# aiforvision/OCTA-autosegmentation

Measured on AMD Instinct MI355X. Metric: synthetic OCTA samples/sec (graph + 304x304 image + 1216x1216 label triples), higher is better.
Workload: dtype f64

## Files before the change

include/octa_hip.h:

```cpp
#ifndef OCTA_HIP_H
#define OCTA_HIP_H

#include <stddef.h>
#include <stdint.h>

#ifdef __cplusplus
extern "C" {
#endif

typedef struct octa_ctx octa_ctx;


int octa_abi_version(void);

const char *octa_last_error(void);

int octa_ctx_create(int device, octa_ctx **out);
void octa_ctx_destroy(octa_ctx *ctx);

size_t octa_ctx_scratch_bytes(const octa_ctx *ctx);

int octa_rasterize_2d(octa_ctx *ctx, int B, const double *d_edges, const int64_t *h_edge_off,
                      const uint8_t *d_keep, int no_pixels_x, int no_pixels_y, int mip_axis,
                      double min_radius, double max_radius, uint8_t *d_out, void *stream);
// ... 129 lines not shown

int octa_menten_vessel_noise(octa_ctx *ctx, const void *d_img, int img_dtype, const unsigned char *d_bernoulli, const double *d_quantum,
                             const double *d_weights, int radius, double scaling, double r, int B, int H, int W, double *d_tmp, double *d_out,
                             void *stream);
int octa_menten_floater_mask(octa_ctx *ctx, const int *d_pts, const int *d_npts, const int *d_dilations, int B, int P, int N,
                             unsigned char *d_mask, int *d_dist, void *stream);
int octa_menten_floater(octa_ctx *ctx, const double *d_img, const int *d_pts, const int *d_npts, const int *d_dilations, const double *d_weights,
                        int radius, int B, int P, int N, unsigned char *d_mask, int *d_dist, double *d_tmp, double *d_out, void *stream);
int octa_menten_motion(octa_ctx *ctx, const void *d_in, void *d_out, int elem_size, const int *d_table, const void *d_white, int n_white,
                       int unit_elems, int B, int H, int W, void *stream);

int octa_noise_model(octa_ctx *ctx, const float *d_img, const float *d_background, const float *d_grids, int B, int H, int W, int gh, int gw,
                     uint64_t seed, uint32_t sample_offset, double lambda_delta, double lambda_speckle, double lambda_gamma,
                     const float *d_delta_in, const float *d_n_in, float *d_out, float *d_maps, float *d_fields, void *stream);
void octa_philox4x32_10(const uint32_t *counter4, const uint32_t *key2, uint32_t *out4);

int octa_noise_model_backward(octa_ctx *ctx, const float *d_dout, const float *d_img, const float *d_background, const float *d_grids, int B, int H,
                              int W, int gh, int gw, uint64_t seed, uint32_t sample_offset, double lambda_delta, double lambda_speckle,
                              double lambda_gamma, const float *d_delta_in, const float *d_n_in, float *d_dgrids, float *d_dmaps, float *d_out,
                              float *d_maps, float *d_logodds, float *d_bgrad, void *stream);

int octa_conv3x3_c1_fwd(octa_ctx *ctx, const void *d_x, const float *d_w, void *d_y, int N, int H, int W, int Cout, double *d_stat, int nslot,
                        void *stream);
int octa_conv3x3_c1_wgrad(octa_ctx *ctx, const void *d_x, const void *d_dy, float *d_dw, int N, int H, int W, int Cout, void *stream);

int octa_dice_bce_fwd(octa_ctx *ctx, const void *d_logits, int dtype, const float *d_y, int B, int64_t n, double *d_sums, void *stream);
int octa_dice_bce_finish(octa_ctx *ctx, const double *d_sums, int B, int64_t n, double smooth_nr, double smooth_dr, float *d_loss, void *stream);
int octa_dice_bce_bwd(octa_ctx *ctx, const void *d_logits, int dtype, const float *d_y, int B, int64_t n, const double *d_sums,
                      const float *d_grad_out, float smooth_nr, float smooth_dr, void *d_dlogits, void *stream);

int octa_thinconv_expand(octa_ctx *ctx, const void *d_s, const void *d_w, const void *d_bias, void *d_out, int N, int Hs, int Ws, int C, int K,
                         int pad, int flip, float slope, void *stream);
int octa_thinconv_squeeze(octa_ctx *ctx, const void *d_a, const void *d_w, const void *d_bias, void *d_out, int N, int Ha, int Wa, int C, int K,
                          int pad, int flip, void *stream);
long long octa_thinconv_wgrad_scratch_floats(int N, int Ha, int C, int K);
int octa_lrelu_bwd_bf16(octa_ctx *ctx, const void *d_y, const void *d_dy, void *d_out, int64_t n, float slope, void *stream);
int octa_thinconv_wgrad(octa_ctx *ctx, const void *d_a, const void *d_s, void *d_scratch, void *d_g, void *d_asum, int N, int Ha, int Wa, int Hs,
                        int Ws, int C, int K, int pad, int flip, void *stream);

int octa_reflect_pad_fwd(octa_ctx *ctx, const void *d_in, void *d_out, int dtype, int B, int H, int W, int C, int pad, void *stream);
int octa_reflect_pad_bwd(octa_ctx *ctx, const void *d_in, void *d_out, int dtype, int B, int H, int W, int C, int pad, void *stream);
int octa_blur_down_fwd(octa_ctx *ctx, const void *d_in, void *d_out, int dtype, int B, int H, int W, int C, void *stream);
int octa_blur_down_bwd(octa_ctx *ctx, const void *d_in, void *d_out, int dtype, int B, int H, int W, int C, void *stream);
int octa_blur_up_fwd(octa_ctx *ctx, const void *d_in, void *d_out, int dtype, int B, int H, int W, int C, void *stream);
int octa_blur_up_bwd(octa_ctx *ctx, const void *d_in, void *d_out, int dtype, int B, int H, int W, int C, void *stream);

int octa_remove_small_objects(octa_ctx *ctx, const uint8_t *d_in, int B, int H, int W, int min_size, int connectivity,
                              uint8_t on_value, uint8_t *d_out, void *stream);

int octa_skeletonize(octa_ctx *ctx, const uint8_t *d_in, int B, int H, int W, uint8_t *d_out, int *passes, void *stream);


size_t octa_fft2_c2c_f64_workspace_bytes(int b, int h, int w);

int octa_fft2_c2c_f64(const void *d_in, void *d_out, int b, int h, int w, int inverse, void *d_ws, void *stream);

size_t octa_oof_workspace_bytes(int b, int h, int w);

int octa_oof_2d(const float *d_in, double *d_out, int b, int h, int w, void *d_ws, void *stream);

int octa_oof_2d_response(const float *d_in, double *d_out, int b, int h, int w, void *d_ws, void *stream);


size_t octa_frangi_workspace_bytes(int b, int h, int w, int n_scales);

int octa_frangi_2d(const float *d_in, double *d_out, int b, int h, int w, int n_scales, const int *radii, const double *weights, float in_scale,
                   double beta, double gamma, int black_ridges, void *d_ws, void *stream);

int octa_frangi_hessian(const float *d_in, float *d_hrr, float *d_hrc, float *d_hcc, int b, int h, int w, int radius, const double *weights,
                        float in_scale, int black_ridges, void *d_ws, void *stream);

int octa_frangi_eigenvalues(const float *d_in, float *d_l1, float *d_l2, float *d_gamma, int b, int h, int w, int radius, const double *weights,
                            float in_scale, int black_ridges, void *d_ws, void *stream);

typedef struct octa_sim octa_sim;

typedef struct {
    double param_scale, d, r;
    double faz_radius_mean, faz_radius_std;
    double rotation_radius;
    double faz_center[2];
    double size[3];
    int n_trees;
    int walls[4];
    int n_modes;
    double modes[8][13];
    int forest_type;
    double nerve_center[2];
    double nerve_radius;
    const uint8_t *geometry;
    int geometry_shape[3];
    int n_source_walls;
    int source_walls[6];
} octa_sim_config;

#define OCTA_BIF_MAX_ATTS 256
typedef struct {
    int sample, n;
    double pos[3];
    double r, kappa, d;
    double atts[OCTA_BIF_MAX_ATTS * 3];
} octa_bif_request;

typedef void (*octa_bif_fn)(int n_req, const octa_bif_request *reqs, double *out6, void *user);

int octa_bif_native_init(const char *blas_path, int n_kappa, const double *kappas, const double *cs, const double *sn,
                         octa_bif_fn fallback, void *fallback_user);
void octa_bif_native(int n_req, const octa_bif_request *reqs, double *out6, void *user);
int octa_bif_native_counts(int64_t *h_out2);

int octa_sim_create(octa_ctx *ctx, const octa_sim_config *cfg, int B, octa_sim **out);
int octa_sim_create_ex(octa_ctx *ctx, const octa_sim_config *cfg, int B, int build, octa_sim **out);
void octa_sim_destroy(octa_sim *sim);

long long octa_sim_launch_count(void);
int octa_order_wait_launch(octa_ctx *ctx, long long ticket, int timeout_us, int settle_us, int *d_out3, void *stream);

int octa_sim_run(octa_sim *sim, const uint32_t *h_np_seeds, const uint64_t *h_py_seeds, octa_bif_fn bif, void *user,
                 void *stream);

int octa_sim_run_states(octa_sim *sim, const double *h_faz_radius, const double *h_stumps, const uint32_t *h_np_states,
                        const uint32_t *h_py_states, octa_bif_fn bif, void *user, void *stream);
int octa_sim_np_state(octa_sim *sim, int sample, uint32_t *h_state625);

int octa_sim_edge_offsets(octa_sim *sim, int64_t *h_edge_off, int64_t *h_n_art);

int octa_sim_export_edges(octa_sim *sim, double *h_edges);

int octa_sim_export_edges_device(octa_sim *sim, double *d_edges, void *stream);

int octa_sim_trace(octa_sim *sim, int32_t *h_trace);

int octa_sim_stats(octa_sim *sim, int64_t *h_stats);

int octa_sim_kd_paths(octa_sim *sim, int64_t *h_paths);

int octa_sim_assign_paths(octa_sim *sim, int64_t *h_paths);

int octa_sim_spans(octa_sim *sim, int64_t *h_spans);

int octa_sim_timing(octa_sim *sim, double *h_out8);

int octa_sim_service_stats(octa_sim *sim, double *h_out5);

int octa_sim_geometry(int num_cus, int *h_out4);

int octa_sim_is_large(const octa_sim *sim);

int octa_sim_fields(octa_sim *sim, int sample, double *h_oxy, int64_t cap_oxy, int64_t *n_oxy, double *h_co2,
                    int64_t cap_co2, int64_t *n_co2);

int octa_sim_kat_kd_order(octa_ctx *ctx, const double *h_pts, int64_t n, const uint8_t *h_need, int32_t *h_indices);

#ifdef __cplusplus
}
#endif
#endif
```

octa_autosegmentation_amd/_native.py:

```python
import contextlib
import ctypes
import os
import random as _random
import threading

import numpy as np

HERE = os.path.dirname(os.path.abspath(__file__))
LIB_PATH = os.environ.get("OCTA_HIP_LIB") or os.path.join(HERE, "liboctahip.so")

_lib = None
_ctxs = {}
_lock = threading.Lock()

c_void_p, c_int, c_double, c_size_t = ctypes.c_void_p, ctypes.c_int, ctypes.c_double, ctypes.c_size_t


def _struct(name, ints, ptrs):
    fields = [("struct_size", ctypes.c_uint32)] + [(k, c_int) for k in ints.split()] + [("slope", ctypes.c_float)] + [(k, c_void_p) for k in ptrs.split()]
    return type(name, (ctypes.Structure,), {"_fields_": fields})


Conv3x3Args = _struct("Conv3x3Args", "N H W Cin Cout stride in_dilation tap_mask out_scale out_off_y out_off_x C1 CY1 nslot",
                      "d_x d_x2 d_w d_y d_y2 d_scale1 d_shift1 d_scale2 d_shift2 d_stat_partials d_stat_slots d_residual")
Conv3x3WgradArgs = _struct("Conv3x3WgradArgs", "N H W Cin Cout stride tap_mask C1 out_mode", "d_x d_x2 d_dy d_dw d_scale1 d_shift1 d_scale2 d_shift2")
WGRAD_TAP_MAJOR, WGRAD_PARAM_ADD, WGRAD_PARAM_SET = 0, 1, 2

SIGNATURES = {
    "octa_abi_version": (c_int, []),
    "octa_last_error": (ctypes.c_char_p, []),
    "octa_ctx_create": (c_int, [c_int, ctypes.POINTER(c_void_p)]),
    "octa_ctx_destroy": (None, [c_void_p]),
    "octa_ctx_scratch_bytes": (c_size_t, [c_void_p]),
    "octa_rasterize_2d": (c_int, [c_void_p, c_int, c_void_p, c_void_p, c_void_p, c_int, c_int, c_int, c_double,
                                  c_double, c_void_p, c_void_p]),
    "octa_rasterize_2d_plan": (c_int, [c_void_p, c_int, c_void_p, c_void_p, c_void_p, c_int, c_int, c_int, c_double, c_double, c_void_p]),
    "octa_rasterize_2d_draw": (c_int, [c_void_p, c_void_p, c_void_p]),
    "octa_raster_prof": (c_int, [c_void_p, c_void_p]),
    "octa_fs_dither": (c_int, [c_void_p, c_int, c_void_p, c_int, c_int, c_void_p, c_void_p]),
    "octa_voxel_padded_dims": (c_int, [c_void_p, c_void_p]),
    "octa_voxelize_3d": (c_int, [c_void_p, c_int, c_void_p, c_void_p, c_void_p, c_void_p, c_double, c_double, c_int, c_void_p, c_void_p]),
    "octa_edges_read_back": (c_int, [c_void_p, c_void_p, c_void_p, ctypes.c_int64, c_void_p, c_void_p]),
    "octa_max_u8": (c_int, [c_void_p, c_void_p, c_void_p, c_void_p, c_size_t, c_void_p]),
    "octa_bif_native_init": (c_int, [ctypes.c_char_p, c_int, c_void_p, c_void_p, c_void_p, c_void_p, c_void_p]),
    "octa_bif_native": (None, [c_int, c_void_p, c_void_p, c_void_p]),
    "octa_bif_native_counts": (c_int, [c_void_p]),
    "octa_instnorm_lrelu_fwd": (c_int, [c_void_p] * 7 + [c_int, c_int, ctypes.c_int64, c_int, ctypes.c_float, ctypes.c_float, c_void_p]),
    "octa_instnorm_lrelu_bwd": (c_int, [c_void_p] * 10 + [c_int, c_int, ctypes.c_int64, c_int, ctypes.c_float, c_void_p]),
    "octa_csv_bytes_bound": (ctypes.c_int64, [ctypes.c_int64]),
    "octa_csv_format_edges": (ctypes.c_int64, [c_void_p, ctypes.c_int64, c_void_p, ctypes.c_int64]),
    "octa_csv_write_file": (c_int, [ctypes.c_char_p, c_void_p, ctypes.c_int64]),
    "octa_csv_count_rows": (ctypes.c_int64, [c_void_p, ctypes.c_int64]),
    "octa_csv_parse_edges": (ctypes.c_int64, [c_void_p, ctypes.c_int64, c_void_p, ctypes.c_int64]),
    "octa_py_random_advance": (c_int, [c_void_p, ctypes.c_int64]),
    "octa_png_write_gray8": (c_int, [ctypes.c_char_p, c_void_p, c_int, c_int, c_int]),
    "octa_png_write_bits": (c_int, [ctypes.c_char_p, c_void_p, c_int, c_int, c_int]),
    "octa_write_sample_files": (c_int, [ctypes.c_int64, c_void_p, c_void_p, c_void_p, c_void_p, c_void_p, c_int, c_int, c_void_p, c_int, c_int, c_int,
                                        ctypes.c_char_p, ctypes.c_int64, c_int, c_int]),
    "octa_pack_bits": (c_int, [c_void_p, c_void_p, c_void_p, ctypes.c_int64, c_int, c_void_p]),
    "octa_background_noise": (c_int, [c_void_p, c_void_p, c_void_p, c_void_p, ctypes.c_int64, c_void_p, c_void_p, c_void_p]),
    "octa_speckle_brightness": (c_int, [c_void_p, c_void_p, c_void_p, c_void_p, c_int, c_int, c_int, c_void_p, c_void_p, c_void_p]),
    "octa_menten_vessel_noise": (c_int, [c_void_p, c_void_p, c_int, c_void_p, c_void_p, c_void_p, c_int, c_double, c_double, c_int, c_int, c_int, c_void_p, c_void_p, c_void_p]),
    "octa_menten_floater_mask": (c_int, [c_void_p, c_void_p, c_void_p, c_void_p, c_int, c_int, c_int, c_void_p, c_void_p, c_void_p]),
    "octa_menten_floater": (c_int, [c_void_p, c_void_p, c_void_p, c_void_p, c_void_p, c_void_p, c_int, c_int, c_int, c_int, c_void_p, c_void_p, c_void_p, c_void_p, c_void_p]),
    "octa_menten_motion": (c_int, [c_void_p, c_void_p, c_void_p, c_int, c_void_p, c_void_p, c_int, c_int, c_int, c_int, c_int, c_void_p]),
    "octa_noise_model": (c_int, [c_void_p, c_void_p, c_void_p, c_void_p, c_int, c_int, c_int, c_int, c_int, ctypes.c_uint64, ctypes.c_uint32, c_double, c_double, c_double,
                                 c_void_p, c_void_p, c_void_p, c_void_p, c_void_p, c_void_p]),
    "octa_noise_model_backward": (c_int, [c_void_p, c_void_p, c_void_p, c_void_p, c_void_p, c_int, c_int, c_int, c_int, c_int, ctypes.c_uint64, ctypes.c_uint32,
                                          c_double, c_double, c_double, c_void_p, c_void_p, c_void_p, c_void_p, c_void_p, c_void_p, c_void_p, c_void_p, c_void_p]),
    "octa_philox4x32_10": (None, [c_void_p, c_void_p, c_void_p]),
    "octa_sim_create": (c_int, [c_void_p, c_void_p, c_int, ctypes.POINTER(c_void_p)]),
    "octa_sim_create_ex": (c_int, [c_void_p, c_void_p, c_int, c_int, ctypes.POINTER(c_void_p)]),
    "octa_sim_destroy": (None, [c_void_p]),
    "octa_sim_run": (c_int, [c_void_p, c_void_p, c_void_p, c_void_p, c_void_p, c_void_p]),
    "octa_sim_run_states": (c_int, [c_void_p, c_void_p, c_void_p, c_void_p, c_void_p, c_void_p, c_void_p, c_void_p]),
    "octa_sim_np_state": (c_int, [c_void_p, c_int, c_void_p]),
    "octa_thinconv_expand": (c_int, [c_void_p, c_void_p, c_void_p, c_void_p, c_void_p, c_int, c_int, c_int, c_int, c_int, c_int, c_int, ctypes.c_float, c_void_p]),
    "octa_thinconv_squeeze": (c_int, [c_void_p, c_void_p, c_void_p, c_void_p, c_void_p, c_int, c_int, c_int, c_int, c_int, c_int, c_int, c_void_p]),
    "octa_lrelu_bwd_bf16": (c_int, [c_void_p, c_void_p, c_void_p, c_void_p, ctypes.c_int64, ctypes.c_float, c_void_p]),
    "octa_thinconv_wgrad_scratch_floats": (ctypes.c_longlong, [c_int, c_int, c_int, c_int]),
    "octa_thinconv_wgrad": (c_int, [c_void_p, c_void_p, c_void_p, c_void_p, c_void_p, c_void_p, c_int, c_int, c_int, c_int, c_int, c_int, c_int, c_int, c_int, c_void_p]),
    "octa_sim_spans": (c_int, [c_void_p, c_void_p]),
    "octa_sim_edge_offsets": (c_int, [c_void_p, c_void_p, c_void_p]),
    "octa_sim_export_edges": (c_int, [c_void_p, c_void_p]),
    "octa_sim_export_edges_device": (c_int, [c_void_p, c_void_p, c_void_p]),
    "octa_sim_trace": (c_int, [c_void_p, c_void_p]),
    "octa_sim_stats": (c_int, [c_void_p, c_void_p]),
    "octa_sim_kd_paths": (c_int, [c_void_p, c_void_p]),
    "octa_sim_assign_paths": (c_int, [c_void_p, c_void_p]),
    "octa_sim_timing": (c_int, [c_void_p, c_void_p]),
    "octa_sim_service_stats": (c_int, [c_void_p, c_void_p]),
    "octa_sim_geometry": (c_int, [c_int, c_void_p]),
    "octa_sim_is_large": (c_int, [c_void_p]),
    "octa_conv2d_f32_nchw": (c_int, [c_void_p, c_void_p, c_void_p, c_void_p, c_void_p] + [c_int] * 14 + [c_void_p]),
    "octa_convtranspose2x2_f32_nchw": (c_int, [c_void_p, c_void_p, c_void_p, c_void_p, c_int, c_int, c_int, c_int, c_int, c_void_p]),
    "octa_conv2d_f32_dgrad_nchw": (c_int, [c_void_p, c_void_p, c_void_p, c_void_p] + [c_int] * 11 + [c_void_p]),
    "octa_conv2d_f32_wgrad_workspace": (c_int, [c_int] * 10 + [ctypes.POINTER(c_size_t)]),
    "octa_conv2d_f32_wgrad_nchw": (c_int, [c_void_p, c_void_p, c_void_p, c_void_p, c_void_p, c_void_p, c_size_t] + [c_int] * 10 + [c_void_p]),
    "octa_sim_fields": (c_int, [c_void_p, c_int, c_void_p, ctypes.c_int64, c_void_p, c_void_p, ctypes.c_int64, c_void_p]),
    "octa_instnorm_lrelu_nhwc_bwd": (c_int, [c_void_p, c_void_p, c_void_p, c_void_p, c_void_p, c_void_p, c_void_p, c_void_p, c_void_p, c_void_p, c_int, c_int, ctypes.c_int64, ctypes.c_float, c_void_p]),
    "octa_pack_conv_weights": (c_int, [c_void_p, c_void_p, c_int, c_void_p, c_void_p]),
    "octa_head1_nhwc_bwd": (c_int, [c_void_p, c_void_p, c_void_p, c_void_p, ctypes.c_int64, c_int, c_void_p, c_void_p, c_void_p, c_void_p]),
    "octa_instnorm_nhwc_stats": (c_int, [c_void_p, c_void_p, c_void_p, c_void_p, c_void_p, c_void_p, c_void_p, c_void_p, c_int, c_int, ctypes.c_int64, ctypes.c_float, c_void_p]),
    "octa_scale_shift_lrelu_nhwc": (c_int, [c_void_p, c_void_p, c_void_p, c_void_p, c_void_p, c_int, c_int, ctypes.c_int64, ctypes.c_float, c_void_p]),
    "octa_resize_bilinear": (c_int, [c_void_p, c_void_p, c_int, c_int, c_int, c_int, c_void_p, c_int, c_int, c_void_p, c_void_p, c_void_p]),
    "octa_resize_bilinear_bwd": (c_int, [c_void_p, c_void_p, c_int, c_int, c_int, c_int, c_int, c_void_p, c_void_p]),
    "octa_flip_rot90_rotate": (c_int, [c_void_p, c_void_p, c_void_p, c_int, c_int, c_void_p, c_void_p, c_void_p, ctypes.c_float, c_int, c_void_p]),
    "octa_remove_small_objects": (c_int, [c_void_p, c_void_p, c_int, c_int, c_int, c_int, c_int, ctypes.c_uint8, c_void_p, c_void_p]),
    "octa_skeletonize": (c_int, [c_void_p, c_void_p, c_int, c_int, c_int, c_void_p, ctypes.POINTER(c_int), c_void_p]),
    "octa_reflect_pad_fwd": (c_int, [c_void_p, c_void_p, c_void_p, c_int, c_int, c_int, c_int, c_int, c_int, c_void_p]),
    "octa_reflect_pad_bwd": (c_int, [c_void_p, c_void_p, c_void_p, c_int, c_int, c_int, c_int, c_int, c_int, c_void_p]),
    "octa_blur_down_fwd": (c_int, [c_void_p, c_void_p, c_void_p, c_int, c_int, c_int, c_int, c_int, c_void_p]),
    "octa_blur_down_bwd": (c_int, [c_void_p, c_void_p, c_void_p, c_int, c_int, c_int, c_int, c_int, c_void_p]),
    "octa_blur_up_fwd": (c_int, [c_void_p, c_void_p, c_void_p, c_int, c_int, c_int, c_int, c_int, c_void_p]),
    "octa_blur_up_bwd": (c_int, [c_void_p, c_void_p, c_void_p, c_int, c_int, c_int, c_int, c_int, c_void_p]),
    "octa_conv4x4_nhwc_fwd": (c_int, [c_void_p, c_void_p, c_void_p, c_void_p, c_int, c_int, c_int, c_int, c_int, c_int, c_void_p]),
    "octa_conv4x4_nhwc_wgrad": (c_int, [c_void_p, c_void_p, c_void_p, c_void_p, c_int, c_int, c_int, c_int, c_int, c_void_p]),
    "octa_dice_bce_fwd": (c_int, [c_void_p, c_void_p, c_int, c_void_p, c_int, ctypes.c_int64, c_void_p, c_void_p]),
    "octa_dice_bce_finish": (c_int, [c_void_p, c_void_p, c_int, ctypes.c_int64, c_double, c_double, c_void_p, c_void_p]),
    "octa_dice_bce_bwd": (c_int, [c_void_p, c_void_p, c_int, c_void_p, c_int, ctypes.c_int64, c_void_p, c_void_p, ctypes.c_float, ctypes.c_float, c_void_p, c_void_p]),
    "octa_sim_launch_count": (ctypes.c_longlong, []),
    "octa_order_wait_launch": (c_int, [c_void_p, ctypes.c_longlong, c_int, c_int, c_void_p, c_void_p]),
    "octa_conv3x3_c1_wgrad": (c_int, [c_void_p, c_void_p, c_void_p, c_void_p, c_int, c_int, c_int, c_int, c_void_p]),
    "octa_conv_stat_tiles": (c_int, [c_int, c_int]),
    "octa_instnorm_lrelu_head1_nhwc_bwd": (c_int, [c_void_p, c_void_p, c_void_p, c_void_p, c_void_p, c_void_p, c_void_p, c_void_p, c_void_p, c_void_p, c_void_p, c_void_p, c_void_p, c_int, c_int, ctypes.c_int64, ctypes.c_float, c_void_p]),
    "octa_conv3x3_s2t_nhwc": (c_int, [c_void_p, c_void_p, c_void_p, c_void_p, c_int, c_int, c_int, c_int, c_int, c_int, c_void_p, c_void_p]),
    "octa_conv3x3_nhwc_fwd": (c_int, [c_void_p, ctypes.POINTER(Conv3x3Args), c_void_p]),
    "octa_conv3x3_nhwc_wgrad": (c_int, [c_void_p, ctypes.POINTER(Conv3x3WgradArgs), c_void_p]),
    "octa_conv3x3_nhwc_fwd_pad": (c_int, [c_void_p, c_void_p, c_void_p, c_void_p, c_int, c_int, c_int, c_int, c_int, c_int, c_int, c_void_p, c_int, c_void_p]),
    "octa_conv3x3_nhwc_wgrad_pad": (c_int, [c_void_p, c_void_p, c_void_p, c_void_p, c_int, c_int, c_int, c_int, c_int, c_int, c_int, c_int, c_void_p]),
    "octa_instnorm_lrelu_nhwc_fwd": (c_int, [c_void_p] * 7 + [c_int, c_int, ctypes.c_int64, ctypes.c_float, ctypes.c_float, c_void_p, c_int, c_void_p, c_int, c_void_p]),
    "octa_instnorm_lrelu_head1_nhwc_fwd": (c_int, [c_void_p] * 9 + [c_int, c_int, ctypes.c_int64, ctypes.c_float, ctypes.c_float, c_void_p, c_int, c_void_p]),
    "octa_head1_nhwc_fwd": (c_int, [c_void_p, c_void_p, c_void_p, c_void_p, ctypes.c_int64, c_int, c_void_p, c_void_p]),
    "octa_conv3x3_c1_fwd": (c_int, [c_void_p, c_void_p, c_void_p, c_void_p, c_int, c_int, c_int, c_int, c_void_p, c_int, c_void_p]),
    "octa_fft2_c2c_f64_workspace_bytes": (c_size_t, [c_int, c_int, c_int]),
    "octa_fft2_c2c_f64": (c_int, [c_void_p, c_void_p, c_int, c_int, c_int, c_int, c_void_p, c_void_p]),
    "octa_oof_workspace_bytes": (c_size_t, [c_int, c_int, c_int]),
    "octa_oof_2d": (c_int, [c_void_p, c_void_p, c_int, c_int, c_int, c_void_p, c_void_p]),
    "octa_oof_2d_response": (c_int, [c_void_p, c_void_p, c_int, c_int, c_int, c_void_p, c_void_p]),
    "octa_frangi_workspace_bytes": (c_size_t, [c_int, c_int, c_int, c_int]),
    "octa_frangi_2d": (c_int, [c_void_p, c_void_p, c_int, c_int, c_int, c_int, c_void_p, c_void_p, ctypes.c_float, c_double, c_double, c_int, c_void_p, c_void_p]),
    "octa_frangi_hessian": (c_int, [c_void_p, c_void_p, c_void_p, c_void_p, c_int, c_int, c_int, c_int, c_void_p, ctypes.c_float, c_int, c_void_p, c_void_p]),
    "octa_frangi_eigenvalues": (c_int, [c_void_p, c_void_p, c_void_p, c_void_p, c_int, c_int, c_int, c_int, c_void_p, ctypes.c_float, c_int, c_void_p, c_void_p]),
    "octa_sim_kat_kd_order": (c_int, [c_void_p, c_void_p, ctypes.c_int64, c_void_p, c_void_p]),
}


class OctaHipError(RuntimeError):
    pass


def lib():
    global _lib
    if _lib is None:
        with _lock:
            if _lib is None:
                if not os.path.exists(LIB_PATH):
                    raise OctaHipError(
                        f"{LIB_PATH} is missing: build it with `python -m octa_autosegmentation_amd.build` "
                        "(hipcc --offload-arch=gfx950). There is no CPU fallback.")
                import torch
                l = ctypes.CDLL(LIB_PATH)
                for name, (res, args) in SIGNATURES.items():
                    fn = getattr(l, name)
                    fn.restype = res
                    fn.argtypes = args
                _lib = l
    return _lib


_SYNC_DEBUG = bool(os.environ.get("OCTA_SYNC_DEBUG"))


def check(rc, what):
    if _SYNC_DEBUG and rc == 0:
        import sys
        import torch
        torch.cuda.current_stream().synchronize()
        print(f"[octa-sync] {threading.current_thread().name} {what} ok", file=sys.stderr, flush=True)
    if rc != 0:
        msg = lib().octa_last_error().decode("utf-8", "replace")
        raise OctaHipError(f"{what} failed (rc={rc}): {msg}")


_tls = threading.local()


def _device_index(device_index):
    import torch
    if not torch.cuda.is_available():
        raise OctaHipError("no ROCm GPU visible to torch; the HIP path cannot run (no CPU fallback)")
    return int(torch.cuda.current_device() if device_index is None else device_index)


def _create_ctx(device_index):
    out = c_void_p()
    call("octa_ctx_create", device_index, ctypes.byref(out))
    return out


def new_ctx(device_index=None):
    return _create_ctx(_device_index(device_index))


def free_ctx(h):
    if h is not None:
        lib().octa_ctx_destroy(h)


@contextlib.contextmanager
def use_ctx(h):
    prev = getattr(_tls, "ctx", None)
    _tls.ctx = h
    try:
        yield h
    finally:
        _tls.ctx = prev


def ctx(device_index=None):
    import torch
    if getattr(_tls, "ctx", None) is not None:
        return _tls.ctx
    device_index = _device_index(device_index)
    key = (device_index, threading.get_ident(), torch.cuda.current_stream(device_index).cuda_stream)
    with _lock:
        h = _ctxs.get(key)
    if h is None:
        h = _create_ctx(device_index)
        with _lock:
            _ctxs[key] = h
    return h


def current_stream_ptr():
    import torch
    return c_void_p(torch.cuda.current_stream().cuda_stream)


def addr(t):
    return t.data_ptr() if t is not None else None


def _ctx_of(device):
    return ctx(device.index)



def launch(name, device, *args, what=None, ctx=None, stream=None):
    argv = [_ctx_of(device) if ctx is None else ctx]
    for a in args:
        argv.append(a.data_ptr() if hasattr(a, "data_ptr") else a)
    argv.append(current_stream_ptr() if stream is None else stream)
    check(getattr(lib(), name)(*argv), what or name)


def call(name, *args, what=None):
    check(getattr(lib(), name)(*[a.data_ptr() if hasattr(a, "data_ptr") else a for a in args]), what or name)


def advance_python_random(n):
    if n <= 0:
        return
    if n < 64:
        for _ in range(n):
            _random.random()
        return
    ver, state, gauss = _random.getstate()
    arr = np.array(state, dtype=np.uint32)
    call("octa_py_random_advance", arr.ctypes.data, int(n))
    _random.setstate((ver, tuple(arr.tolist()), gauss))
```

octa_autosegmentation_amd/csrc/sim.hip:

```cpp

#include <chrono>
#include <vector>

#include "common.h"
#include "sim_host.h"
#include <thread>
#include <atomic>
#include <cstdlib>
#include <cstring>

using namespace OCTA_SIMK;

#if OCTA_SIM_LARGE
#define OCTA_SIM_T octa_simL_impl
#define OCTA_SIM_FN(name) octa_simL_##name
#else
#define OCTA_SIM_T octa_simS_impl
#define OCTA_SIM_FN(name) octa_simS_##name
#endif
#define octa_sim_create OCTA_SIM_FN(create)
#define octa_sim_destroy OCTA_SIM_FN(destroy)
#define octa_sim_run OCTA_SIM_FN(run)
#define octa_sim_run_states OCTA_SIM_FN(run_states)
#define octa_sim_np_state OCTA_SIM_FN(np_state)
#define octa_sim_edge_offsets OCTA_SIM_FN(edge_offsets)
#define octa_sim_export_edges OCTA_SIM_FN(export_edges)
#define octa_sim_export_edges_device OCTA_SIM_FN(export_edges_device)
#define octa_sim_trace OCTA_SIM_FN(trace)
#define octa_sim_stats OCTA_SIM_FN(stats)
#define octa_sim_kd_paths OCTA_SIM_FN(kd_paths)
#define octa_sim_assign_paths OCTA_SIM_FN(assign_paths)
#define octa_sim_fields OCTA_SIM_FN(fields)
#define octa_sim_service_stats OCTA_SIM_FN(service_stats)
#define octa_sim_geometry OCTA_SIM_FN(geometry)
#define octa_sim_spans OCTA_SIM_FN(spans)
#define octa_sim_timing OCTA_SIM_FN(timing)
#define octa_sim_kat_kd_order OCTA_SIM_FN(kat_kd_order)
struct OCTA_SIM_T;
extern "C" void octa_sim_destroy(OCTA_SIM_T *S);
extern "C" long long octa_sim_next_ticket(void);
extern "C" int *octa_sim_launch_flag(int device);

namespace {

constexpr int SIM_THREADS = SIM_THREADS_PER_WG;
constexpr int SIM_WG_PER_CU = 2;
#if OCTA_SIM_LARGE
constexpr size_t SIM_LDS = 2048;
#else
constexpr size_t SIM_LDS = SIM_LDS_BYTES;
static_assert((size_t)KD_MAILBOX_OFF + KD_MAILBOX_BYTES <= (size_t)SIM_USER_BYTES && SIM_WG_PER_CU * SIM_LDS <= 160 * 1024, "LDS budget");
#endif
static_assert((624 + 1248) * 4 <= SEQ_SIDE_LDS, "the Mersenne-Twister state and queue of the candidate stream fit the side-job LDS");
static_assert(SIM_THREADS == 64 * KD_WAVES, "kd mailboxes are sized for KD_WAVES waves");
constexpr int REQ_CAP = 8192;

static_assert(sizeof(BifRequest) == sizeof(octa_bif_request), "request layout must match the public header");
static_assert(MAXKEPT == OCTA_BIF_MAX_ATTS, "request capacity must match the public header");

struct BatchPtrs {
    double *npos[2], *nrad[2], *nkap[2];
    int *npar[2], *nch0[2], *nch1[2];
    unsigned char *nnch[2], *nact[2];
    double *oxy, *co2, *cand, *py_u;
    unsigned *py_state;
    int *nn, *act_list;
    int *nn_prev[2];
    double *nn_d2[2];
    unsigned *sorted;
    int *gnode, *gstart, *gcount;
    Rec *rec;
    int *glist, *child_group;
    FlushRec *fl_rec;
    idx_t *kd_idx, *kd_rank;
    unsigned char *removed, *ven_near;
    unsigned long long *hashes;
    unsigned *pairs;
    unsigned long long *set_hash;
    int *set_key, *tmp_int;
    double *grid_pts;
    unsigned *cand_idx;
    double *tmp_dbl;
    SampleScalars *sc;
    IterParams *iters;
    BifRequest *reqs;
    int *req_count;
    double *bif_results;
    unsigned *mt_state;
    unsigned short *valid;
    size_t valid_stride;
    unsigned *valid_count;
    int *n_per_iter;
    int *next_sample;
    unsigned char *wg_scratch;
#ifdef OCTA_SIM_DEBUG_SAT
    int *dbg;
#endif
    int *trace;
    int n_samples;
    SimConst C;
};

__device__ __forceinline__ SimArrays sample_arrays(const BatchPtrs &B, int s) {
    SimArrays A;
    for (int f = 0; f < 2; f++) {
        A.npos[f] = B.npos[f] + (size_t)s * NCAP * 3;
        A.nrad[f] = B.nrad[f] + (size_t)s * NCAP;
        A.nkap[f] = B.nkap[f] + (size_t)s * NCAP;
        A.npar[f] = B.npar[f] + (size_t)s * NCAP;
        A.nch0[f] = B.nch0[f] + (size_t)s * NCAP;
        A.nch1[f] = B.nch1[f] + (size_t)s * NCAP;
        A.nnch[f] = B.nnch[f] + (size_t)s * NCAP;
        A.nact[f] = B.nact[f] + (size_t)s * NCAP;
        A.nn_prev[f] = B.nn_prev[f] + (size_t)s * OCAP;
        A.nn_d2[f] = B.nn_d2[f] + (size_t)s * OCAP;
    }
    A.oxy = B.oxy + (size_t)s * OCAP * 3;
    A.co2 = B.co2 + (size_t)s * CCAP * 3;
    A.cand = B.cand + (size_t)s * NCANDCAP * 3;
    A.py_u = B.py_u + (size_t)s * PYCAP;
    A.nn = B.nn + (size_t)s * OCAP;
    A.act_list = B.act_list + (size_t)s * NCAP;
    A.sorted = B.sorted + (size_t)s * SORTCAP;
    A.gnode = B.gnode + (size_t)s * GCAP;
    A.gstart = B.gstart + (size_t)s * GCAP;
    A.gcount = B.gcount + (size_t)s * GCAP;
    A.rec = B.rec + (size_t)s * GCAP;
    A.glist = B.glist + (size_t)s * GCAP;
    A.child_group = B.child_group + (size_t)s * NCAP;
    A.fl_rec = B.fl_rec + (size_t)s * 2 * MURRAY_FLUSH_LDS;
    A.kd_idx = B.kd_idx + (size_t)s * OCAP;
    A.kd_rank = B.kd_rank + (size_t)s * OCAP;
    A.removed = B.removed + (size_t)s * OCAP;
    A.ven_near = B.ven_near + (size_t)s * OCAP;
    A.hashes = B.hashes + (size_t)s * OCAP;
    A.pairs = B.pairs + (size_t)s * PCAP;
    A.set_hash = B.set_hash + (size_t)s * SETCAP;
    A.set_key = B.set_key + (size_t)s * SETCAP;
    A.tmp_int = B.tmp_int + (size_t)s * (OCAP + 2 * NCANDCAP);
    A.grid_pts = B.grid_pts + (size_t)s * GRID_N * 3;
    A.tmp_dbl = B.tmp_dbl + (size_t)s * OCAP * 3;
    A.sc = B.sc + s;
#ifdef OCTA_SIM_DEBUG_SAT
    A.dbg = B.dbg ? B.dbg + (size_t)s * B.C.n_iter * 16 : nullptr;
    A.dbg_it = 0;
#endif
    return A;
}

struct WaveMt {
    unsigned *st;
    unsigned *ob;
    int cur, avail;
    int lane;
    __device__ void regen_block() {
        for (int c = 0; c < 623; c += 64) {
            int k = c + lane;
            unsigned nv = 0;
            if (k < 623) {
                unsigned y = (st[k] & 0x80000000u) | (st[k + 1] & 0x7fffffffu);
                unsigned m = (k < 227) ? st[k + 397] : st[k - 227];
                nv = m ^ (y >> 1) ^ ((y & 1u) ? 0x9908b0dfu : 0u);
            }
            __builtin_amdgcn_wave_barrier();
            if (k < 623) st[k] = nv;
            __builtin_amdgcn_wave_barrier();
        }
        if (lane == 0) {
            unsigned y = (st[623] & 0x80000000u) | (st[0] & 0x7fffffffu);
            st[623] = st[396] ^ (y >> 1) ^ ((y & 1u) ? 0x9908b0dfu : 0u);
        }
        __builtin_amdgcn_wave_barrier();
    }
    __device__ static unsigned temper(unsigned y) {
        y ^= (y >> 11);
        y ^= (y << 7) & 0x9d2c5680u;
        y ^= (y << 15) & 0xefc60000u;
        y ^= (y >> 18);
        return y;
    }
    __device__ void ensure(int k) {
        if (avail - cur >= k) return;
        const int rem = avail - cur;
        for (int c = 0; c < rem; c += 64) {
            int i = c + lane;
            unsigned v = (i < rem) ? ob[cur + i] : 0u;
            __builtin_amdgcn_wave_barrier();
            if (i < rem) ob[i] = v;
            __builtin_amdgcn_wave_barrier();
        }
// ... 942 lines not shown
            OCTA_HIP_CHECK(hipEventSynchronize(S->ev[1]));
            OCTA_HIP_CHECK(hipEventElapsedTime(&ms, S->ev[0], S->ev[1]));
            S->ms_a += ms; S->n_a++;
            break;
        }
        if (serve(0)) return -1;
        OCTA_HIP_CHECK(hipEventElapsedTime(&ms, S->ev[0], S->ev[1]));
        S->ms_a += ms; S->n_a++;
        OCTA_HIP_CHECK(hipEventRecord(S->ev[0], stream));
        hipLaunchKernelGGL(sim_iter_b_kernel, dim3((unsigned)B), dim3(SIM_THREADS), SIM_LDS, stream, P, it);
        OCTA_HIP_CHECK(hipGetLastError());
        OCTA_HIP_CHECK(hipEventRecord(S->ev[1], stream));
        if (serve(1)) return -1;
        OCTA_HIP_CHECK(hipEventElapsedTime(&ms, S->ev[0], S->ev[1]));
        S->ms_b += ms; S->n_b++;
    }
    S->ms_total = std::chrono::duration<double, std::milli>(std::chrono::steady_clock::now() - wall0).count();
    if (S->lockstep) {
        S->h_sc.resize(B);
        OCTA_HIP_CHECK(hipMemcpyAsync(S->h_sc.data(), P.sc, sizeof(SampleScalars) * B, hipMemcpyDeviceToHost, stream));
        OCTA_HIP_CHECK(hipStreamSynchronize(stream));
    }
    S->ran = true;
#ifdef OCTA_SIM_DEBUG_SAT
    if (const char *path = getenv("OCTA_SIM_DEBUG_DUMP")) {
        std::vector<int> h((size_t)B * S->iters.size() * 16);
        OCTA_HIP_CHECK(hipMemcpy(h.data(), P.dbg, h.size() * sizeof(int), hipMemcpyDeviceToHost));
        if (FILE *fp = fopen(path, "wb")) { fwrite(h.data(), sizeof(int), h.size(), fp); fclose(fp); }
    }
#endif
    for (int s = 0; s < B; s++)
        if (S->h_sc[s].err) {
            if ((S->h_sc[s].err & ERR_HOST_TIMEOUT) && !S->lockstep)
                octa::set_error("octa_sim_run: sample %d failed with capacity/error bits 0x%x: with parking disabled (OCTA_SIM_PARK_MS=0) a workgroup waited "
                                "more than %.0f ms for the host's mailbox answer (request ticket %d, answered %d, %ld tickets served this run, longest pass of the "
                                "service loop %.1f ms, longest bifurcation callback %.1f ms; the workgroup began waiting for ticket %ld at %.1f ms into its "
                                "launch, polled %ld times, at its deadline read answer %ld and its own request word back as %ld)", s, S->h_sc[s].err,
                                S->mail_timeout_ms, S->mail.req_ticket[s], S->mail.resp_ticket[s], S->diag_tickets, S->diag_max_gap_ms, S->diag_max_bif_ms,
                                S->h_sc[s].prof[13], S->h_sc[s].prof[12] * 1e-5, S->h_sc[s].prof[14], S->h_sc[s].prof[11], S->h_sc[s].prof[15]);
            else
                octa::set_error("octa_sim_run: sample %d failed with capacity/error bits 0x%x", s, S->h_sc[s].err);
            return -3;
        }
    return 0;
}
}

extern "C" int octa_sim_edge_offsets(OCTA_SIM_T *S, int64_t *h_edge_off, int64_t *h_n_art) {
    if (!S || !S->ran || !h_edge_off) { octa::set_error("octa_sim_edge_offsets: run the simulation first"); return -2; }
    h_edge_off[0] = 0;
    for (int s = 0; s < S->B; s++) {
        const SampleScalars &sc = S->h_sc[s];
        int64_t na = sc.n_nodes[0] - S->cfg.n_trees, nv = sc.n_nodes[1] - S->cfg.n_trees;
        h_edge_off[s + 1] = h_edge_off[s] + na + nv;
        if (h_n_art) h_n_art[s] = na;
    }
    return 0;
}

extern "C" int octa_sim_export_edges(OCTA_SIM_T *S, double *h_edges) {
    if (!S || !S->ran || !h_edges) { octa::set_error("octa_sim_export_edges: run the simulation first"); return -2; }
    OCTA_HIP_CHECK(hipSetDevice(S->ctx->device));
    const BatchPtrs &P = S->P;
    const int B = S->B;
    int nmax[2] = {0, 0};
    for (int s = 0; s < B; s++) for (int f = 0; f < 2; f++) nmax[f] = S->h_sc[s].n_nodes[f] > nmax[f] ? S->h_sc[s].n_nodes[f] : nmax[f];
    size_t need = 0;
    for (int f = 0; f < 2; f++) need += (size_t)B * nmax[f] * (24 + 8 + 4 + 4 + 4 + 1) + 64 * 6;
    if (S->export_cap < need) {
        if (S->export_stage) { hipError_t e = hipHostFree(S->export_stage); (void)e; S->export_stage = nullptr; S->export_cap = 0; }
        OCTA_HIP_CHECK(hipHostMalloc(&S->export_stage, need + need / 4));
        S->export_cap = need + need / 4;
    }
    hipStream_t stream = S->export_stream;
    if (!stream) { OCTA_HIP_CHECK(hipStreamCreateWithFlags(&S->export_stream, hipStreamNonBlocking)); stream = S->export_stream; }
    char *base = static_cast<char *>(S->export_stage);
    double *pos[2], *rad[2];
    int *par[2], *c0[2], *c1[2];
    unsigned char *nch[2];
    size_t off = 0;
    auto take = [&](size_t bytes) { char *p = base + off; off += (bytes + 63) & ~(size_t)63; return p; };
    for (int f = 0; f < 2; f++) {
        const size_t n = (size_t)nmax[f];
        pos[f] = reinterpret_cast<double *>(take((size_t)B * n * 24)); rad[f] = reinterpret_cast<double *>(take((size_t)B * n * 8));
        par[f] = reinterpret_cast<int *>(take((size_t)B * n * 4)); c0[f] = reinterpret_cast<int *>(take((size_t)B * n * 4));
        c1[f] = reinterpret_cast<int *>(take((size_t)B * n * 4)); nch[f] = reinterpret_cast<unsigned char *>(take((size_t)B * n));
        if (n == 0) continue;
        auto get = [&](void *dst, const void *src, size_t elem, size_t cap_elems) -> hipError_t {
            return hipMemcpy2DAsync(dst, n * elem, src, cap_elems * elem, n * elem, (size_t)B, hipMemcpyDeviceToHost, stream);
        };
        OCTA_HIP_CHECK(get(pos[f], P.npos[f], 24, NCAP)); OCTA_HIP_CHECK(get(rad[f], P.nrad[f], 8, NCAP));
        OCTA_HIP_CHECK(get(par[f], P.npar[f], 4, NCAP)); OCTA_HIP_CHECK(get(c0[f], P.nch0[f], 4, NCAP));
        OCTA_HIP_CHECK(get(c1[f], P.nch1[f], 4, NCAP)); OCTA_HIP_CHECK(get(nch[f], P.nnch[f], 1, NCAP));
    }
    OCTA_HIP_CHECK(hipStreamSynchronize(stream));
    long total = 0;
    for (int s = 0; s < B; s++) {
        const SampleScalars &sc = S->h_sc[s];
        const double *cp[2], *cr[2];
        const int *cpar[2], *cc0[2], *cc1[2];
        const unsigned char *cn[2];
        for (int f = 0; f < 2; f++) {
            const size_t n = (size_t)nmax[f];
            cp[f] = pos[f] + (size_t)s * n * 3; cr[f] = rad[f] + (size_t)s * n; cpar[f] = par[f] + (size_t)s * n;
            cc0[f] = c0[f] + (size_t)s * n; cc1[f] = c1[f] + (size_t)s * n; cn[f] = nch[f] + (size_t)s * n;
        }
        long n_art = 0;
        long ne = export_edges(cp, cr, cpar, cc0, cc1, cn, sc.n_nodes, S->cfg.n_trees, h_edges + 7 * total, 1L << 40, &n_art);
        if (ne < 0) { octa::set_error("octa_sim_export_edges: export failed"); return -1; }
        total += ne;
    }
    return 0;
}

extern "C" int octa_sim_export_edges_device(OCTA_SIM_T *S, double *d_edges, void *stream_) {
    if (!S || !S->ran || !d_edges) { octa::set_error("octa_sim_export_edges_device: run the simulation first"); return -2; }
    OCTA_HIP_CHECK(hipSetDevice(S->ctx->device));
    hipStream_t stream = (hipStream_t)stream_;
    const int B = S->B;
    std::vector<long> off(B + 1, 0);
    for (int s = 0; s < B; s++) off[s + 1] = off[s] + (S->h_sc[s].n_nodes[0] - S->cfg.n_trees) + (S->h_sc[s].n_nodes[1] - S->cfg.n_trees);
    if (!S->d_edge_off) OCTA_HIP_CHECK(hipMalloc(&S->d_edge_off, sizeof(long) * (B + 1)));
    OCTA_HIP_CHECK(hipMemcpyAsync(S->d_edge_off, off.data(), sizeof(long) * (B + 1), hipMemcpyHostToDevice, stream));
    OCTA_HIP_CHECK(hipStreamSynchronize(stream));
    const size_t lds = OCTA_SIM_LARGE ? 2048 : 2048 + (size_t)NCAP * 2 * sizeof(idx_t);
    hipLaunchKernelGGL(sim_export_kernel, dim3((unsigned)B, 2), dim3(256), lds, stream, S->P, S->d_edge_off, S->cfg.n_trees, d_edges);
    OCTA_HIP_CHECK(hipGetLastError());
    return 0;
}

extern "C" int octa_sim_trace(OCTA_SIM_T *S, int32_t *h_trace) {
    if (!S || !S->ran || !h_trace) { octa::set_error("octa_sim_trace: run the simulation first"); return -2; }
    OCTA_HIP_CHECK(hipSetDevice(S->ctx->device));
    OCTA_HIP_CHECK(hipMemcpy(h_trace, S->P.trace, sizeof(int32_t) * (size_t)S->B * S->iters.size() * 4, hipMemcpyDeviceToHost));
    return 0;
}

extern "C" int octa_sim_stats(OCTA_SIM_T *S, int64_t *h_stats) {
    if (!S || !S->ran || !h_stats) { octa::set_error("octa_sim_stats: run the simulation first"); return -2; }
    for (int s = 0; s < S->B; s++) {
        const SampleScalars &sc = S->h_sc[s];
        int64_t *o = h_stats + 32 * s;
        o[0] = sc.err; o[1] = sc.py_pos; o[2] = sc.murray_steps; o[3] = sc.n_bif; o[4] = sc.respec;
        o[5] = sc.n_nodes[0]; o[6] = sc.n_nodes[1];
        memcpy(&o[7], &sc.faz_radius, 8);
        for (int k = 0; k < 16; k++) o[8 + k] = sc.prof[k];
        for (int k = 0; k < 8; k++) o[24 + k] = sc.kdprof[k];
    }
    return 0;
}

extern "C" int octa_sim_kd_paths(OCTA_SIM_T *S, int64_t *h_paths) {
    if (!S || !S->ran || !h_paths) { octa::set_error("octa_sim_kd_paths: run the simulation first"); return -2; }
    for (int s = 0; s < S->B; s++) { h_paths[2 * s] = S->h_sc[s].kd_path[0]; h_paths[2 * s + 1] = S->h_sc[s].kd_path[1]; }
    return 0;
}

extern "C" int octa_sim_assign_paths(OCTA_SIM_T *S, int64_t *h_paths) {
    if (!S || !S->ran || !h_paths) { octa::set_error("octa_sim_assign_paths: run the simulation first"); return -2; }
    for (int s = 0; s < S->B; s++) { h_paths[2 * s] = S->h_sc[s].assign_path[0]; h_paths[2 * s + 1] = S->h_sc[s].assign_path[1]; }
    return 0;
}

extern "C" int octa_sim_fields(OCTA_SIM_T *S, int sample, double *h_oxy, int64_t cap_oxy, int64_t *n_oxy, double *h_co2,
                               int64_t cap_co2, int64_t *n_co2) {
    if (!S || !S->ran || sample < 0 || sample >= S->B) { octa::set_error("octa_sim_fields: bad arguments"); return -2; }
    OCTA_HIP_CHECK(hipSetDevice(S->ctx->device));
    const SampleScalars &sc = S->h_sc[sample];
    if (n_oxy) *n_oxy = sc.n_oxy;
    if (n_co2) *n_co2 = sc.n_co2;
    if (h_oxy) {
        int64_t n = sc.n_oxy < cap_oxy ? sc.n_oxy : cap_oxy;
        OCTA_HIP_CHECK(hipMemcpy(h_oxy, S->P.oxy + (size_t)sample * OCAP * 3, sizeof(double) * 3 * n, hipMemcpyDeviceToHost));
    }
    if (h_co2) {
        int64_t n = sc.n_co2 < cap_co2 ? sc.n_co2 : cap_co2;
        OCTA_HIP_CHECK(hipMemcpy(h_co2, S->P.co2 + (size_t)sample * CCAP * 3, sizeof(double) * 3 * n, hipMemcpyDeviceToHost));
    }
    return 0;
}

#if !OCTA_SIM_LARGE
namespace {
__global__ void __launch_bounds__(SIM_THREADS)
sim_kat_kd_kernel(const double *pts, int n, const unsigned char *need, idx_t *out_idx, idx_t *out_rank, float *xy, double zlo, double zhi) {
    extern __shared__ __attribute__((aligned(16))) unsigned char smem[];
    Blk b = {(int)threadIdx.x, (int)blockDim.x, smem};
    kd_build(b, pts, n, out_idx, out_rank, xy, zlo, zhi, nullptr, need);
}
}

extern "C" int octa_sim_kat_kd_order(octa_ctx *ctx, const double *h_pts, int64_t n, const uint8_t *h_need, int32_t *h_indices) {
    if (!ctx || !h_pts || !h_indices || n < 0 || n > OCAP) { octa::set_error("octa_sim_kat_kd_order: bad arguments"); return -2; }
    if (n == 0) return 0;
    OCTA_HIP_CHECK(hipSetDevice(ctx->device));
    double *d_pts = nullptr;
    unsigned char *d_need = nullptr;
    idx_t *d_idx = nullptr;
    float *d_xy = nullptr;
    double zlo = h_pts[2], zhi = h_pts[2];
    for (int64_t i = 1; i < n; i++) { zlo = h_pts[3 * i + 2] < zlo ? h_pts[3 * i + 2] : zlo; zhi = h_pts[3 * i + 2] > zhi ? h_pts[3 * i + 2] : zhi; }
    OCTA_HIP_CHECK(hipMalloc(&d_xy, sizeof(float) * 2 * n));
    OCTA_HIP_CHECK(hipMalloc(&d_pts, sizeof(double) * 3 * n));
    OCTA_HIP_CHECK(hipMalloc(&d_idx, sizeof(idx_t) * 2 * n));
    OCTA_HIP_CHECK(hipMemcpy(d_pts, h_pts, sizeof(double) * 3 * n, hipMemcpyHostToDevice));
    if (h_need) {
        OCTA_HIP_CHECK(hipMalloc(&d_need, n));
        OCTA_HIP_CHECK(hipMemcpy(d_need, h_need, n, hipMemcpyHostToDevice));
    }
    OCTA_HIP_CHECK(hipFuncSetAttribute(reinterpret_cast<const void *>(sim_kat_kd_kernel), hipFuncAttributeMaxDynamicSharedMemorySize, (int)SIM_LDS));
    hipLaunchKernelGGL(sim_kat_kd_kernel, dim3(1), dim3(SIM_THREADS), SIM_LDS, 0, d_pts, (int)n, d_need, d_idx, d_idx + n, d_xy, zlo, zhi);
    OCTA_HIP_CHECK(hipGetLastError());
    std::vector<idx_t> h(n);
    OCTA_HIP_CHECK(hipMemcpy(h.data(), d_idx, sizeof(idx_t) * n, hipMemcpyDeviceToHost));
    for (int64_t i = 0; i < n; i++) h_indices[i] = (int32_t)h[i];
    (void)hipFree(d_pts); (void)hipFree(d_idx); (void)hipFree(d_xy); if (d_need) (void)hipFree(d_need);
    return 0;
}

#endif

extern "C" int octa_sim_service_stats(OCTA_SIM_T *S, double *h_out4) {
    if (!S || !S->ran || !h_out4) { octa::set_error("octa_sim_service_stats: run the simulation first"); return -2; }
    h_out4[0] = (double)S->diag_tickets; h_out4[1] = S->diag_max_gap_ms; h_out4[2] = (double)S->diag_relaunches; h_out4[3] = (double)S->diag_parked;
    h_out4[4] = S->diag_max_bif_ms;
    return 0;
}

extern "C" int octa_sim_geometry(int num_cus, int *h_out4) {
    if (!h_out4) { octa::set_error("octa_sim_geometry: null output"); return -2; }
    h_out4[0] = SIM_THREADS; h_out4[1] = SIM_WG_PER_CU; h_out4[2] = (int)SIM_LDS; h_out4[3] = SIM_WG_PER_CU * (num_cus > 0 ? num_cus : 256);
    return 0;
}

extern "C" int octa_sim_spans(OCTA_SIM_T *S, int64_t *h_spans) {
    if (!S || !S->ran || !h_spans) { octa::set_error("octa_sim_spans: run the simulation first"); return -2; }
    for (int s = 0; s < S->B; s++) { h_spans[2 * s] = S->h_sc[s].t_begin; h_spans[2 * s + 1] = S->h_sc[s].t_end; }
    return 0;
}

extern "C" int octa_sim_timing(OCTA_SIM_T *S, double *h_out8) {
    if (!S || !S->ran || !h_out8) { octa::set_error("octa_sim_timing: run the simulation first"); return -2; }
    h_out8[0] = S->ms_a; h_out8[1] = (double)S->n_a; h_out8[2] = S->ms_b; h_out8[3] = (double)S->n_b;
    h_out8[4] = S->ms_total; h_out8[5] = S->ms_host_bif; h_out8[6] = (double)S->n_bif_req; h_out8[7] = (double)S->bytes;
    return 0;
}
```

octa_autosegmentation_amd/csrc/sim_api.cpp:

```cpp
#include <cstdlib>
#include <cstring>
#include <new>

#include "common.h"

extern "C" {
struct octa_simS_impl;
struct octa_simL_impl;
#define OCTA_DECL(SFX, T)                                                                                                                       \
    int octa_sim##SFX##_create(octa_ctx *, const octa_sim_config *, int, T **);                                                                 \
    void octa_sim##SFX##_destroy(T *);                                                                                                          \
    int octa_sim##SFX##_run(T *, const uint32_t *, const uint64_t *, octa_bif_fn, void *, void *);                                              \
    int octa_sim##SFX##_run_states(T *, const double *, const double *, const uint32_t *, const uint32_t *, octa_bif_fn, void *, void *);       \
    int octa_sim##SFX##_np_state(T *, int, uint32_t *);                                                                                         \
    int octa_sim##SFX##_edge_offsets(T *, int64_t *, int64_t *);                                                                                \
    int octa_sim##SFX##_export_edges(T *, double *);                                                                                            \
    int octa_sim##SFX##_export_edges_device(T *, double *, void *);                                                                             \
    int octa_sim##SFX##_trace(T *, int32_t *);                                                                                                  \
    int octa_sim##SFX##_stats(T *, int64_t *);                                                                                                  \
    int octa_sim##SFX##_kd_paths(T *, int64_t *);                                                                                               \
    int octa_sim##SFX##_assign_paths(T *, int64_t *);                                                                                           \
    int octa_sim##SFX##_spans(T *, int64_t *);                                                                                                  \
    int octa_sim##SFX##_timing(T *, double *);                                                                                                  \
    int octa_sim##SFX##_service_stats(T *, double *);                                                                                           \
    int octa_sim##SFX##_geometry(int, int *);                                                                                                   \
    int octa_sim##SFX##_fields(T *, int, double *, int64_t, int64_t *, double *, int64_t, int64_t *);
OCTA_DECL(S, octa_simS_impl)
OCTA_DECL(L, octa_simL_impl)
#undef OCTA_DECL
int octa_simS_kat_kd_order(octa_ctx *, const double *, int64_t, const uint8_t *, int32_t *);
}

#include <atomic>
#include <mutex>
static std::atomic<long long> g_sim_launches{0};
extern "C" long long octa_sim_next_ticket(void) { return g_sim_launches.fetch_add(1, std::memory_order_acq_rel) + 1; }
extern "C" long long octa_sim_launch_count(void) { return g_sim_launches.load(std::memory_order_acquire); }
extern "C" int *octa_sim_launch_flag(int device) {
    static std::mutex m;
    static int *flags[64] = {};
    if (device < 0 || device >= 64) return nullptr;
    std::lock_guard<std::mutex> g(m);
    if (!flags[device]) {
        int prev = 0;
        if (hipGetDevice(&prev) != hipSuccess || hipSetDevice(device) != hipSuccess) return nullptr;
        int *p = nullptr;
        if (hipMalloc(&p, 64) != hipSuccess || hipMemset(p, 0, 64) != hipSuccess || hipDeviceSynchronize() != hipSuccess) { (void)hipSetDevice(prev); return nullptr; }
        (void)hipSetDevice(prev);
        flags[device] = p;
    }
    return flags[device];
}

struct octa_sim {
    bool large = false;
    octa_simS_impl *s = nullptr;
    octa_simL_impl *l = nullptr;
};

static bool wants_large(const octa_sim_config *c) {
    if (const char *e = getenv("OCTA_SIM_BUILD")) {
        if (!strcmp(e, "large")) return true;
        if (!strcmp(e, "default")) return false;
    }
    if (c->param_scale <= 6.0) return false;
    int iters = 0, nmax = 0;
    for (int m = 0; m < c->n_modes && m < 8; m++) {
        const int I = (int)c->modes[m][0], N = (int)c->modes[m][1];
        if (I > 0) { iters += I; nmax = N > nmax ? N : nmax; }
    }
    return nmax > 8192 / 3 && iters > 40;
}

#define FWD(call_s, call_l) (sim->large ? (call_l) : (call_s))

extern "C" int octa_sim_create_ex(octa_ctx *ctx, const octa_sim_config *cfg, int B, int build, octa_sim **out) {
    if (!out || !cfg || build < 0 || build > 2) { octa::set_error("octa_sim_create: bad arguments"); return -2; }
    *out = nullptr;
    octa_sim *sim = new (std::nothrow) octa_sim();
    if (!sim) { octa::set_error("octa_sim_create: out of host memory"); return -1; }
    sim->large = build == 0 ? wants_large(cfg) : build == 2;
    const int rc = sim->large ? octa_simL_create(ctx, cfg, B, &sim->l) : octa_simS_create(ctx, cfg, B, &sim->s);
    if (rc) { delete sim; return rc; }
    *out = sim;
    return 0;
}
extern "C" int octa_sim_create(octa_ctx *ctx, const octa_sim_config *cfg, int B, octa_sim **out) { return octa_sim_create_ex(ctx, cfg, B, 0, out); }
extern "C" void octa_sim_destroy(octa_sim *sim) {
    if (!sim) return;
    if (sim->large) octa_simL_destroy(sim->l); else octa_simS_destroy(sim->s);
    delete sim;
}
#define NEED(sim, what) if (!(sim)) { octa::set_error(what ": null simulator"); return -2; }
extern "C" int octa_sim_run(octa_sim *sim, const uint32_t *a, const uint64_t *b, octa_bif_fn f, void *u, void *st) {
    NEED(sim, "octa_sim_run") return FWD(octa_simS_run(sim->s, a, b, f, u, st), octa_simL_run(sim->l, a, b, f, u, st));
}
extern "C" int octa_sim_run_states(octa_sim *sim, const double *fz, const double *stp, const uint32_t *a, const uint32_t *b, octa_bif_fn f, void *u, void *st) {
    NEED(sim, "octa_sim_run_states") return FWD(octa_simS_run_states(sim->s, fz, stp, a, b, f, u, st), octa_simL_run_states(sim->l, fz, stp, a, b, f, u, st));
}
extern "C" int octa_sim_np_state(octa_sim *sim, int k, uint32_t *o) { NEED(sim, "octa_sim_np_state") return FWD(octa_simS_np_state(sim->s, k, o), octa_simL_np_state(sim->l, k, o)); }
extern "C" int octa_sim_edge_offsets(octa_sim *sim, int64_t *a, int64_t *b) { NEED(sim, "octa_sim_edge_offsets") return FWD(octa_simS_edge_offsets(sim->s, a, b), octa_simL_edge_offsets(sim->l, a, b)); }
extern "C" int octa_sim_export_edges(octa_sim *sim, double *e) { NEED(sim, "octa_sim_export_edges") return FWD(octa_simS_export_edges(sim->s, e), octa_simL_export_edges(sim->l, e)); }
extern "C" int octa_sim_export_edges_device(octa_sim *sim, double *e, void *st) {
    NEED(sim, "octa_sim_export_edges_device") return FWD(octa_simS_export_edges_device(sim->s, e, st), octa_simL_export_edges_device(sim->l, e, st));
}
extern "C" int octa_sim_trace(octa_sim *sim, int32_t *t) { NEED(sim, "octa_sim_trace") return FWD(octa_simS_trace(sim->s, t), octa_simL_trace(sim->l, t)); }
extern "C" int octa_sim_stats(octa_sim *sim, int64_t *t) { NEED(sim, "octa_sim_stats") return FWD(octa_simS_stats(sim->s, t), octa_simL_stats(sim->l, t)); }
extern "C" int octa_sim_kd_paths(octa_sim *sim, int64_t *t) { NEED(sim, "octa_sim_kd_paths") return FWD(octa_simS_kd_paths(sim->s, t), octa_simL_kd_paths(sim->l, t)); }
extern "C" int octa_sim_assign_paths(octa_sim *sim, int64_t *t) { NEED(sim, "octa_sim_assign_paths") return FWD(octa_simS_assign_paths(sim->s, t), octa_simL_assign_paths(sim->l, t)); }
extern "C" int octa_sim_spans(octa_sim *sim, int64_t *t) { NEED(sim, "octa_sim_spans") return FWD(octa_simS_spans(sim->s, t), octa_simL_spans(sim->l, t)); }
extern "C" int octa_sim_timing(octa_sim *sim, double *t) { NEED(sim, "octa_sim_timing") return FWD(octa_simS_timing(sim->s, t), octa_simL_timing(sim->l, t)); }
extern "C" int octa_sim_service_stats(octa_sim *sim, double *t) { NEED(sim, "octa_sim_service_stats") return FWD(octa_simS_service_stats(sim->s, t), octa_simL_service_stats(sim->l, t)); }
extern "C" int octa_sim_fields(octa_sim *sim, int k, double *o, int64_t co, int64_t *no, double *c, int64_t cc, int64_t *nc) {
    NEED(sim, "octa_sim_fields") return FWD(octa_simS_fields(sim->s, k, o, co, no, c, cc, nc), octa_simL_fields(sim->l, k, o, co, no, c, cc, nc));
}
extern "C" int octa_sim_geometry(int num_cus, int *h_out4) { return octa_simS_geometry(num_cus, h_out4); }
extern "C" int octa_sim_kat_kd_order(octa_ctx *ctx, const double *p, int64_t n, const uint8_t *need, int32_t *o) { return octa_simS_kat_kd_order(ctx, p, n, need, o); }
extern "C" int octa_sim_is_large(const octa_sim *sim) { return sim && sim->large ? 1 : 0; }
```

octa_autosegmentation_amd/csrc/sim_core.h:

```cpp
#pragma once
#include <cmath>
#include <cstdint>
#include <cstring>
#include <algorithm>
#include "gpow.h"
#include "glibc_trig.h"

#ifndef OCTA_SIM_LARGE
#define OCTA_SIM_LARGE 0
#endif
#if OCTA_SIM_LARGE
#define OCTA_SIMK octa_simk_large
#else
#define OCTA_SIMK octa_simk
#endif
namespace OCTA_SIMK {

#if OCTA_SIM_LARGE
typedef unsigned int idx_t;
typedef unsigned long long kdw_t;
constexpr int IDX_BITS = 18;
constexpr int GROUP_BITS = 17;
constexpr int NCAP = 1 << 17;
constexpr int OCAP = 1 << 18;
constexpr int CCAP = OCAP;
constexpr int GCAP = 1 << 17;
constexpr int SORTCAP = OCAP;
constexpr int PCAP = 1 << 21;
constexpr int SETCAP = 1 << 20;
constexpr int PYCAP = 1 << 20;
constexpr int ACCCAP = 8192;
constexpr int GRID_MAX = 448;
constexpr int SIM_USER_BYTES = 12 << 20;
constexpr int LSET_PAIRS = 1 << 14, LSET_CAP = 1 << 18;
#else
typedef unsigned short idx_t;
typedef unsigned int kdw_t;
constexpr int IDX_BITS = 14;
constexpr int GROUP_BITS = 13;
constexpr int NCAP = 14336;
constexpr int OCAP = 13312;
constexpr int CCAP = OCAP;
constexpr int GCAP = 8192;
constexpr int SORTCAP = 16384;
constexpr int PCAP = 16384;
constexpr int SETCAP = 16384;
constexpr int PYCAP = 32768;
constexpr int ACCCAP = 2048;
constexpr int GRID_MAX = 112;
constexpr int SIM_USER_BYTES = 78 * 1024;
constexpr int LSET_PAIRS = 512, LSET_CAP = 4096;
#endif
static_assert(OCAP <= (1 << IDX_BITS) && GCAP <= (1 << GROUP_BITS) && NCAP <= (1 << 30), "index widths");
constexpr unsigned IDX_MASK = (1u << IDX_BITS) - 1u;
constexpr idx_t IDX_NONE = (idx_t)~(idx_t)0;
constexpr int MAXKEPT = 256;
constexpr int NCANDCAP = 8192;
constexpr int TILE = 1024;
constexpr int KD_RANGES = OCAP / 17 + 1;
constexpr int KD_TAB_BYTES_PER_RANGE = 4 * (int)sizeof(idx_t) + 1;
constexpr int KD_MAILBOX_OFF = OCAP * (int)sizeof(kdw_t) + ((KD_RANGES * KD_TAB_BYTES_PER_RANGE + 15) / 16) * 16;
constexpr int KD_TEAM_MIN = 192;
#ifndef OCTA_SIM_THREADS
#define OCTA_SIM_THREADS 256
#endif
constexpr int SIM_THREADS_PER_WG = OCTA_SIM_THREADS;
constexpr int KD_WAVES = SIM_THREADS_PER_WG / 64;
constexpr int KD_MAILBOX_BYTES = (OCAP / 2 + 64) * (int)sizeof(idx_t);
constexpr int SIM_LDS_BYTES = SIM_USER_BYTES + 2048;

enum ErrBits { ERR_NODE_CAP = 1, ERR_OXY_CAP = 2, ERR_CO2_CAP = 4, ERR_GROUP_CAP = 8, ERR_PAIR_CAP = 16, ERR_SET_CAP = 32,
               ERR_PY_CAP = 64, ERR_KEPT_CAP = 128, ERR_REQ_CAP = 256, ERR_ACC_CAP = 512, ERR_MISSING_BIF = 1024 };

struct IterParams {
    int t, first_mode, N, pad;
    double eps_n, eps_s, eps_k, delta_art, delta_ven, d, gamma_art, gamma_ven, phi, omega, kappa;
};

struct SimConst {
    double ps, r, rotation_radius, fc0, fc1, sx, sy, sz;
    double gs;
    int n_iter, n_max;
    int fixed;
    int gshape[3];
    const unsigned char *mask;
};

struct __attribute__((aligned(8))) Rec {
    double newpos[3];
    double thr;
    double r1_used;
    int node;
    int req;
    unsigned char type;
    unsigned char draw;
    unsigned char ang_gt90;
    unsigned char grow;
    unsigned int child;
};

struct __attribute__((aligned(8))) FlushRec { double kk, acc; int node, pend, s0, s1; };

struct __attribute__((aligned(8))) BifRequest {
    int sample, n;
    double pos[3];
    double r, kappa, d;
    double atts[MAXKEPT * 3];
};

struct SampleScalars {
    double faz_radius;
    int n_nodes[2];
    int n_oxy, n_co2;
    int py_pos, py_cap;
    int err;
    int new_begin[2], new_end[2];
    int n_groups[2];
    int n_sorted[2];
    int n_grow[2];
    int pass_tag[2];
    int pass_counter;
    long murray_steps;
    long flush_rounds;
    long murray_deferred;
    long n_bif;
    long respec;
    long prof[16];
    long kdprof[8];
    int kd_path[2];
    int resume_it, resume_stage;
    int parked, finished;
    long t_begin, t_end;
    int fl_pending[2];
    int n_cached[2], n_nodes_cached[2];
    double delta_cached[2];
    long assign_path[2];
};

struct SimArrays {
    double *npos[2];
    double *nrad[2];
    double *nkap[2];
    int *npar[2], *nch0[2], *nch1[2];
    unsigned char *nnch[2], *nact[2];
    OCTA_HD double *npos_of(int f) const { return f ? npos[1] : npos[0]; }
    OCTA_HD double *nrad_of(int f) const { return f ? nrad[1] : nrad[0]; }
    OCTA_HD double *nkap_of(int f) const { return f ? nkap[1] : nkap[0]; }
    OCTA_HD int *npar_of(int f) const { return f ? npar[1] : npar[0]; }
    OCTA_HD int *nch0_of(int f) const { return f ? nch0[1] : nch0[0]; }
    OCTA_HD int *nch1_of(int f) const { return f ? nch1[1] : nch1[0]; }
    OCTA_HD unsigned char *nnch_of(int f) const { return f ? nnch[1] : nnch[0]; }
    OCTA_HD unsigned char *nact_of(int f) const { return f ? nact[1] : nact[0]; }
    double *oxy;
    double *co2;
    const double *cand;
    const double *py_u;
    int *nn;
    int *nn_prev[2] = {nullptr, nullptr};
    double *nn_d2[2] = {nullptr, nullptr};
    OCTA_HD int *nn_prev_of(int f) const { return f ? nn_prev[1] : nn_prev[0]; }
    OCTA_HD double *nn_d2_of(int f) const { return f ? nn_d2[1] : nn_d2[0]; }
    int *act_list;
    unsigned *sorted;
    int *gnode, *gstart, *gcount;
    Rec *rec;
    int *glist;
    int *child_group;
    FlushRec *fl_rec;
    idx_t *kd_idx, *kd_rank;
    unsigned char *removed;
    unsigned char *ven_near;
    unsigned long long *hashes;
    unsigned *pairs;
    unsigned long long *set_hash;
    int *set_key;
    double *grid_pts;
    int *tmp_int;
    double *tmp_dbl;
    SampleScalars *sc;
#ifdef OCTA_SIM_DEBUG_SAT
    int *dbg;
    int dbg_it;
#endif
};

#define OCTA_ISSUE_LOADS() asm volatile("" ::: "memory")
#if defined(__HIP_DEVICE_COMPILE__)
#define OCTA_UNI(x) __builtin_amdgcn_readfirstlane(x)
#else
#define OCTA_UNI(x) (x)
#endif

#ifndef OCTA_SIM_SYNC_DRAIN
#define OCTA_SIM_SYNC_DRAIN 1
#endif
#if defined(__HIPCC__)
__device__ __forceinline__ void octa_block_sync() {
#if defined(__HIP_DEVICE_COMPILE__)
#if OCTA_SIM_SYNC_DRAIN & 4
    __builtin_amdgcn_fence(__ATOMIC_RELEASE, "agent");
    __builtin_amdgcn_s_barrier();
    __builtin_amdgcn_fence(__ATOMIC_ACQUIRE, "agent");
    return;
#endif
#if OCTA_SIM_SYNC_DRAIN & 1
#if defined(OCTA_SIM_SYNC_NO_LGKM)
    asm volatile("s_waitcnt vmcnt(0)" ::: "memory");
#elif defined(OCTA_SIM_SYNC_NO_VM)
    asm volatile("s_waitcnt lgkmcnt(0)" ::: "memory");
#else
    asm volatile("s_waitcnt vmcnt(0) lgkmcnt(0)" ::: "memory");
#endif
#endif
    __syncthreads();
#if OCTA_SIM_SYNC_DRAIN & 2
    asm volatile("buffer_inv sc0" ::: "memory");
#endif
#if OCTA_SIM_SYNC_DRAIN & 8
    asm volatile("buffer_inv sc1" ::: "memory");
#endif
#endif
}
#endif

#ifndef OCTA_SIM_DS_MASK
#define OCTA_SIM_DS_MASK 0
#endif
#ifndef OCTA_SIM_DUP
#define OCTA_SIM_DUP 0
#endif
struct Blk {
    int tid, nth;
    unsigned char *smem;
    unsigned char *umem = nullptr;
    mutable unsigned scan_calls = 0;
    OCTA_HD inline void sync() const {
#if defined(__HIP_DEVICE_COMPILE__)
        octa_block_sync();
#endif
    }
    OCTA_HD inline int *coll() const { return reinterpret_cast<int *>(smem); }
#if !OCTA_SIM_LARGE && !defined(OCTA_SIM_FLAT_USER)
    OCTA_HD inline unsigned char *user() const { return smem + 2048; }
#else
    OCTA_HD inline unsigned char *user() const { return umem ? umem : smem + 2048; }
#endif
    template <int TENANT>
    OCTA_HD inline unsigned char *user_of() const {
#if !OCTA_SIM_LARGE
        if (OCTA_SIM_DS_MASK & TENANT) return smem + 2048;
#endif
        return user();
    }
};

#if defined(__HIP_DEVICE_COMPILE__)
__device__ __forceinline__ int wave_scan_incl(int v) {
    v += __builtin_amdgcn_update_dpp(0, v, 0x111, 0xf, 0xf, true);
    v += __builtin_amdgcn_update_dpp(0, v, 0x112, 0xf, 0xf, true);
    v += __builtin_amdgcn_update_dpp(0, v, 0x114, 0xf, 0xf, true);
    v += __builtin_amdgcn_update_dpp(0, v, 0x118, 0xf, 0xf, true);
    v += __builtin_amdgcn_update_dpp(0, v, 0x142, 0xa, 0xf, false);
    v += __builtin_amdgcn_update_dpp(0, v, 0x143, 0xc, 0xf, false);
    return v;
}
#endif

OCTA_HD inline int blk_scan(const Blk &b, int v, int *excl) {
#if defined(__HIP_DEVICE_COMPILE__)
    const int lane = b.tid & 63, wv = b.tid >> 6, nw = (b.nth + 63) >> 6;
    const int inc = wave_scan_incl(v);
    int *sh = b.coll() + ((b.scan_calls++ & 1u) ? 16 : 0);
    if (lane == 63 || b.tid == b.nth - 1) sh[wv] = inc;
    b.sync();
    int base = 0, tot = 0;
    for (int k = 0; k < nw; k++) { const int t = sh[k]; base += k < wv ? t : 0; tot += t; }
    *excl = base + inc - v;
    return OCTA_UNI(tot);
#else
    (void)b;
    *excl = 0;
    return v;
// ... 121 lines not shown
OCTA_HD inline void st3(double *p, V3 v) { p[0] = v.x; p[1] = v.y; p[2] = v.z; }
OCTA_HD inline V3 sub(V3 a, V3 b) { return v3(a.x - b.x, a.y - b.y, a.z - b.z); }
OCTA_HD inline V3 add(V3 a, V3 b) { return v3(a.x + b.x, a.y + b.y, a.z + b.z); }
OCTA_HD inline V3 mul(V3 a, double s) { return v3(a.x * s, a.y * s, a.z * s); }
OCTA_HD inline V3 divs(V3 a, double s) { return v3(a.x / s, a.y / s, a.z / s); }
OCTA_HD inline double norm3(V3 v) { return sqrt(fma(v.z, v.z, fma(v.y, v.y, v.x * v.x))); }
OCTA_HD inline double norm2(double a, double c) { return sqrt(fma(c, c, a * a)); }
OCTA_HD inline double dot3_blas(V3 a, V3 c) { return fma(a.z, c.z, fma(a.y, c.y, a.x * c.x)); }
OCTA_HD inline double dot2_blas(double a0, double a1, double b0, double b1) { return fma(a1, b1, a0 * b0); }
OCTA_HD inline V3 unit(V3 v) { return divs(v, norm3(v)); }
OCTA_HD inline double rownorm(V3 v) { return sqrt((v.x * v.x + v.y * v.y) + v.z * v.z); }
OCTA_HD inline V3 cross(V3 a, V3 c) { return v3(a.y * c.z - a.z * c.y, a.z * c.x - a.x * c.z, a.x * c.y - a.y * c.x); }
OCTA_HD inline double sqdist(V3 a, V3 c) {
    double dx = a.x - c.x, dy = a.y - c.y, dz = a.z - c.z;
    return (dx * dx + dy * dy) + dz * dz;
}
OCTA_HD inline double clip1(double c) { return fmin(fmax(c, -1.0), 1.0); }
OCTA_HD inline double rad2deg() { return 180.0 / 3.14159265358979323846; }
OCTA_HD inline double deg2rad() { return 3.14159265358979323846 / 180.0; }
OCTA_HD inline double angle_uv(V3 u, double nu, V3 v) {
    double c = ((u.x * v.x + u.y * v.y) + u.z * v.z) / nu / rownorm(v);
    return acos(clip1(c)) * rad2deg();
}
OCTA_HD inline double angle2(double u0, double u1, double v0, double v1) {
    double c = dot2_blas(u0, u1, v0, v1) / norm2(u0, u1) / norm2(v0, v1);
    return acos(clip1(c)) * rad2deg();
}
OCTA_HD inline double oxygen_distance(double rad, double ps) {
    const double c_oxygen = 203.9e-3, kap = 0.02 * c_oxygen, r0 = 3.5e-3;
    double q = rad * ps / r0;
    double c1 = kap * q * exp(1 - q);
    return c1 * 6 / ps;
}

OCTA_HD inline unsigned long long py_hash_double(double v) {
    const unsigned long long MOD = (1ULL << 61) - 1;
    int e;
    double m = frexp(v, &e);
    int sign = 1;
    if (m < 0) { sign = -1; m = -m; }
    unsigned long long x = 0;
    while (m != 0.0) {
        x = ((x << 28) & MOD) | x >> (61 - 28);
        m *= 268435456.0;
        e -= 28;
        unsigned long long y = (unsigned long long)m;
        m -= (double)y;
        x += y;
        if (x >= MOD) x -= MOD;
    }
    e = e >= 0 ? e % 61 : 61 - 1 - ((-1 - e) % 61);
    x = ((x << e) & MOD) | x >> (61 - e);
    if (sign < 0) x = 0ULL - x;
    if (x == ~0ULL) x = ~0ULL - 1;
    return x;
}
OCTA_HD inline unsigned long long py_hash_tuple3(V3 t) {
    const unsigned long long P1 = 11400714785074694791ULL, P2 = 14029467366897019727ULL, P5 = 2870177450012600261ULL;
    unsigned long long acc = P5;
    double c[3] = {t.x, t.y, t.z};
    for (int i = 0; i < 3; i++) {
        acc += py_hash_double(c[i]) * P2;
        acc = (acc << 31) | (acc >> 33);
        acc *= P1;
    }
    acc += 3ULL ^ (P5 ^ 3527539ULL);
    if (acc == ~0ULL) return 1546275796ULL;
    return acc;
}

struct PySetView {
    unsigned long long *hash;
    int *key;
    int mask, fill, used;
    int *err;
    int cap;
    int lane = 0, nl = 1;
};
OCTA_HD inline void pyset_team_sync(const PySetView &s) {
#if defined(__HIP_DEVICE_COMPILE__)
    if (s.nl > 1) __builtin_amdgcn_wave_barrier();
#else
    (void)s;
#endif
}
OCTA_HD inline void pyset_init(PySetView &s) {
    for (int i = 0; i < 8; i++) s.key[i] = -1;
    s.mask = 7; s.fill = 0; s.used = 0;
}
OCTA_HD inline void pyset_insert_clean(unsigned long long *h, int *k, int mask, int key, unsigned long long hash) {
    unsigned long long perturb = hash;
    unsigned long long i = hash & (unsigned long long)mask;
    while (true) {
        unsigned long long e = i;
        int probes = (i + 9 <= (unsigned long long)mask) ? 9 : 0;
        do {
            if (k[e] < 0) { k[e] = key; h[e] = hash; return; }
            e++;
        } while (probes--);
        perturb >>= 5;
        i = (i * 5 + 1 + perturb) & (unsigned long long)mask;
    }
}
OCTA_HD inline void pyset_resize(PySetView &s, int minused) {
    int newsize = 8;
    while (newsize <= minused) newsize <<= 1;
    if (newsize > s.cap / 2) { atomic_or_int(s.err, ERR_SET_CAP); return; }
    unsigned long long *nh = s.hash + s.cap / 2;
    int *nk = s.key + s.cap / 2;
    for (int i = s.lane; i < newsize; i += s.nl) nk[i] = -1;
    pyset_team_sync(s);
    for (int base = 0; base <= s.mask; base += s.nl) {
        const int slot = base + s.lane;
        const bool used = slot <= s.mask && s.key[slot] >= 0;
#if defined(__HIP_DEVICE_COMPILE__)
        unsigned long long m = s.nl > 1 ? __ballot(used) : (used ? 1ull : 0ull);
        while (m) {
            const int j = (int)__ffsll((long long)m) - 1;
            m &= m - 1ull;
            pyset_insert_clean(nh, nk, newsize - 1, s.key[base + j], s.hash[base + j]);
        }
#else
        if (used) pyset_insert_clean(nh, nk, newsize - 1, s.key[slot], s.hash[slot]);
#endif
    }
    pyset_team_sync(s);
    for (int i = s.lane; i < newsize; i += s.nl) { s.key[i] = nk[i]; s.hash[i] = nh[i]; }
    pyset_team_sync(s);
    s.mask = newsize - 1;
    s.fill = s.used;
}
OCTA_HD inline void pyset_add(PySetView &s, int key, unsigned long long hash) {
    unsigned long long perturb = hash;
    unsigned long long i = hash & (unsigned long long)s.mask;
    while (true) {
        unsigned long long e = i;
        int probes = (i + 9 <= (unsigned long long)s.mask) ? 9 : 0;
        do {
            if (s.key[e] < 0) {
                s.fill++; s.used++;
                s.key[e] = key; s.hash[e] = hash;
                if (!OCTA_UNLIKELY(!((long)s.fill * 5 < (long)s.mask * 3))) return;
                pyset_resize(s, s.used > 50000 ? s.used * 2 : s.used * 4);
                return;
            }
            if (s.hash[e] == hash && s.key[e] == key) return;
            e++;
        } while (probes--);
        perturb >>= 5;
        i = (i * 5 + 1 + perturb) & (unsigned long long)s.mask;
    }
}

OCTA_HD inline bool pyset_order_free(const int *dk, const int *dg, const unsigned long long *hashes, int D, int *own, int *ord0, int *ord1,
                                     int s_max) {
    int S = 8, n_prev = 0;
    int *ord = ord0, *ord_next = ord1;
    while (true) {
        const int thr = (3 * (S - 1) + 4) / 5;
        const int upto = D < thr ? D : thr;
        const unsigned long long mask = (unsigned long long)(S - 1);
        for (int p = n_prev; p < upto; p++) ord[p] = p;
        for (int e = 0; e < S; e++) own[e] = -1;
        for (int p = 0; p < upto; p++) {
            const int k = ord[p];
            const unsigned long long hsh = hashes[dk[k]];
            unsigned long long perturb = hsh, i = hsh & mask;
            while (true) {
                unsigned long long e = i;
                int probes = (i + 9 <= mask) ? 9 : 0;
                bool placed = false;
                do {
                    const int q = own[e];
                    if (q < 0) { own[e] = p; placed = true; break; }
                    if (p >= n_prev && q >= n_prev && dg[q] == dg[k]) return false;
                    e++;
                } while (probes--);
                if (placed) break;
                perturb >>= 5;
                i = (i * 5 + 1 + perturb) & mask;
            }
        }
        if (D < thr) return true;
        if (D > thr && dg[thr - 1] == dg[thr]) return false;
        const int minused = upto > 50000 ? upto * 2 : upto * 4;
        int newS = 8;
        while (newS <= minused) newS <<= 1;
        if (newS > s_max) return false;
        int c = 0;
        for (int e = 0; e < S; e++) if (own[e] >= 0) ord_next[c++] = ord[own[e]];
        { int *t = ord; ord = ord_next; ord_next = t; }
        n_prev = upto;
        S = newS;
    }
}

constexpr int KD_IDX_BITS = IDX_BITS;
constexpr kdw_t KD_IDX_MASK = ((kdw_t)1 << KD_IDX_BITS) - 1u;
constexpr kdw_t KD_QMAX = ((kdw_t)1 << (8 * (int)sizeof(kdw_t) - KD_IDX_BITS)) - 1u;
static_assert(OCAP <= (1 << KD_IDX_BITS), "kd index bits");
struct KdPair {
    kdw_t *kv;
    const double *pts;
    int d;
};
OCTA_HD inline bool kd_less_w(const KdPair &a, kdw_t x, kdw_t y) {
    if (!OCTA_UNLIKELY(!((x ^ y) >> KD_IDX_BITS))) return x < y;
    const unsigned xi = (unsigned)(x & KD_IDX_MASK), yi = (unsigned)(y & KD_IDX_MASK);
    const double fx = a.pts[3 * xi + a.d], fy = a.pts[3 * yi + a.d];
    if (fx == fy) return xi < yi;
    return fx < fy;
}
OCTA_HD inline bool kd_less(const KdPair &a, int i, int j) { return kd_less_w(a, a.kv[i], a.kv[j]); }
OCTA_HD inline void kd_swap(const KdPair &a, int i, int j) { kdw_t t = a.kv[i]; a.kv[i] = a.kv[j]; a.kv[j] = t; }
OCTA_HD inline kdw_t kd_quant(double x, double mn, double scale) {
    const double t = (x - mn) * scale;
    if (!(t > 0.0)) return 0;
    if (t >= (double)KD_QMAX) return KD_QMAX;
    return (kdw_t)t;
}
OCTA_HD inline void kd_push_heap(const KdPair &a, int first, int hole, int top, kdw_t v) {
    int parent = (hole - 1) / 2;
    while (hole > top && kd_less_w(a, a.kv[first + parent], v)) {
        a.kv[first + hole] = a.kv[first + parent];
        hole = parent;
        parent = (hole - 1) / 2;
    }
    a.kv[first + hole] = v;
}
OCTA_HD inline void kd_adjust_heap(const KdPair &a, int first, int hole, int len, kdw_t v) {
    const int top = hole;
    int second = hole;
    while (second < (len - 1) / 2) {
        second = 2 * (second + 1);
        if (kd_less(a, first + second, first + (second - 1))) second--;
        a.kv[first + hole] = a.kv[first + second];
        hole = second;
    }
    if ((len & 1) == 0 && second == (len - 2) / 2) {
        second = 2 * (second + 1);
        a.kv[first + hole] = a.kv[first + (second - 1)];
        hole = second - 1;
    }
    kd_push_heap(a, first, hole, top, v);
}
OCTA_HD inline void kd_heap_select(const KdPair &a, int first, int middle, int last) {
    int len = middle - first;
    if (len >= 2) {
        int parent = (len - 2) / 2;
        while (true) {
            kdw_t v = a.kv[first + parent];
            kd_adjust_heap(a, first, parent, len, v);
            if (parent == 0) break;
            parent--;
        }
    }
    for (int i = middle; i < last; ++i)
        if (kd_less(a, i, first)) {
            kdw_t v = a.kv[i];
            a.kv[i] = a.kv[first];
            kd_adjust_heap(a, first, 0, middle - first, v);
        }
}
OCTA_HD inline void kd_insertion_sort(const KdPair &a, int first, int last) {
    if (first == last) return;
    for (int i = first + 1; i < last; ++i) {
        const kdw_t v = a.kv[i];
        if (kd_less_w(a, v, a.kv[first])) {
            for (int k = i; k > first; --k) a.kv[k] = a.kv[k - 1];
            a.kv[first] = v;
        } else {
            int lastp = i, next = i - 1;
            while (kd_less_w(a, v, a.kv[next])) {
                a.kv[lastp] = a.kv[next];
                lastp = next; --next;
            }
            a.kv[lastp] = v;
        }
    }
}
OCTA_HD inline void kd_median_to_first(const KdPair &a, int first, int last) {
    const int mid = first + (last - first) / 2;
    const int A = first + 1, B = mid, C = last - 1;
    if (kd_less(a, A, B)) {
        if (kd_less(a, B, C)) kd_swap(a, first, B);
        else if (kd_less(a, A, C)) kd_swap(a, first, C);
        else kd_swap(a, first, A);
    } else if (kd_less(a, A, C)) kd_swap(a, first, A);
    else if (kd_less(a, B, C)) kd_swap(a, first, C);
    else kd_swap(a, first, B);
}
OCTA_HD inline void kd_nth_element(const KdPair &a, int first, int nth, int last) {
    if (first == last || nth == last) return;
    int n = last - first, lg = 0;
    while ((n >> (lg + 1)) > 0) lg++;
    int depth = lg * 2;
    while (last - first > 3) {
        if (depth == 0) {
            kd_heap_select(a, first, nth + 1, last);
            kd_swap(a, first, nth);
            return;
        }
        --depth;
        kd_median_to_first(a, first, last);
        int lo = first + 1, hi = last;
        while (true) {
            while (kd_less(a, lo, first)) ++lo;
            --hi;
            while (kd_less(a, first, hi)) --hi;
            if (!(lo < hi)) break;
            kd_swap(a, lo, hi);
            ++lo;
        }
        int cut = lo;
        if (cut <= nth) first = cut; else last = cut;
    }
    kd_insertion_sort(a, first, last);
}


#if defined(__HIP_DEVICE_COMPILE__)
template <int TW, int NW>
__device__ inline void kd_nth_element_team(const KdPair &a, int first, int nth, int last, bool live,
                                           idx_t *mb, int depth_left = -1) {
    const int tl = (int)(threadIdx.x & (TW - 1));
    if (!live || first == last || nth == last) return;
    idx_t *box = mb + ((first + 1) >> 1);
    int n = last - first, lg = 0;
    while ((n >> (lg + 1)) > 0) lg++;
    int depth = depth_left >= 0 ? depth_left : lg * 2;
    while (last - first > 3) {
        if (OCTA_UNLIKELY(depth == 0)) {
            if (tl == 0) { kd_heap_select(a, first, nth + 1, last); kd_swap(a, first, nth); }
            __builtin_amdgcn_wave_barrier();
            return;
        }
        --depth;
        kdw_t pk;
        {
            const int iA = first + 1, iB = first + (last - first) / 2, iC = last - 1;
            const kdw_t x0 = a.kv[first], xa = a.kv[iA], xb = a.kv[iB], xc = a.kv[iC];
            const bool ab = kd_less_w(a, xa, xb), bc = kd_less_w(a, xb, xc), ac = kd_less_w(a, xa, xc);
            const int im = ab ? (bc ? iB : (ac ? iC : iA)) : (ac ? iA : (bc ? iC : iB));
            pk = im == iA ? xa : (im == iB ? xb : xc);
            __builtin_amdgcn_wave_barrier();
            if (tl == 0) { a.kv[first] = pk; a.kv[im] = x0; }
        }
// ... 32 lines not shown
            inc += __builtin_amdgcn_update_dpp(0, inc, 0x112, 0xf, 0xf, true);
            inc += __builtin_amdgcn_update_dpp(0, inc, 0x114, 0xf, 0xf, true);
            inc += __builtin_amdgcn_update_dpp(0, inc, 0x118, 0xf, 0xf, true);
            totS = __shfl(inc, TW - 1, TW);
        }
        const int preS = inc - nS;
        const int cut = base + totS;
        {
            int g = (p0 - base) - preS;
#pragma unroll
            for (int w = 0; w < NW; w++) {
                const int q0 = p0 + 64 * w;
                int lim = ((p1 < cut) ? p1 : cut) - q0;
                if (lim <= 0) continue;
                unsigned long long inv = ~ms[w];
                if (lim < 64) inv &= (1ull << lim) - 1ull;
                while (inv) {
                    int i = (int)__ffsll((long long)inv) - 1;
                    inv &= inv - 1ull;
                    box[g++] = (idx_t)(q0 + i);
                }
            }
        }
        __builtin_amdgcn_wave_barrier();
        {
            int r = totS - preS - nS;
#pragma unroll
            for (int w = NW - 1; w >= 0; w--) {
                const int q0 = p0 + 64 * w;
                if (q0 >= p1) continue;
                unsigned long long sm = ms[w];
                if (cut > q0) { int sh = cut - q0; sm = (sh >= 64) ? 0ull : (sm >> sh) << sh; }
                while (sm) {
                    int i = 63 - __clzll((long long)sm);
                    sm &= ~(1ull << i);
                    kd_swap(a, q0 + i, (int)box[r++]);
                }
            }
        }
        __builtin_amdgcn_wave_barrier();
        if (cut <= nth) first = cut; else last = cut;
    }
    if (tl == 0) kd_insertion_sort(a, first, last);
    __builtin_amdgcn_wave_barrier();
}
constexpr int KD_MASK_MAX = 16000;
__device__ inline void kd_nth_element_wave_long(const KdPair &a, int first, int nth, int last, idx_t *mb) {
    const int tl = (int)(threadIdx.x & 63);
    if (first == last || nth == last) return;
    idx_t *box = mb + ((first + 1) >> 1);
    int n = last - first, lg = 0;
    while ((n >> (lg + 1)) > 0) lg++;
    int depth = lg * 2;
    while (last - first > KD_MASK_MAX) {
        if (depth == 0) {
            if (tl == 0) { kd_heap_select(a, first, nth + 1, last); kd_swap(a, first, nth); }
            __builtin_amdgcn_wave_barrier();
            return;
        }
        --depth;
        if (tl == 0) kd_median_to_first(a, first, last);
        __builtin_amdgcn_wave_barrier();
        const kdw_t pk = a.kv[first];
        const int base = first + 1, m = last - base;
        const int c = ((m + 63) / 64) | 1;
        int p0 = base + tl * c;
        if (p0 > last) p0 = last;
        const int p1 = (p0 + c < last) ? p0 + c : last;
        int nS = 0;
        for (int i = p0; i < p1; i++) nS += kd_less_w(a, a.kv[i], pk) ? 1 : 0;
        int inc = nS;
#pragma unroll
        for (int d = 1; d < 64; d <<= 1) {
            int u = __shfl_up(inc, d, 64);
            if (tl >= d) inc += u;
        }
        const int totS = __shfl(inc, 63, 64);
        const int preS = inc - nS;
        const int cut = base + totS;
        {
            int g = (p0 - base) - preS;
            const int lim = p1 < cut ? p1 : cut;
            for (int i = p0; i < lim; i++)
                if (!kd_less_w(a, a.kv[i], pk)) box[g++] = (idx_t)i;
        }
        __builtin_amdgcn_wave_barrier();
        {
            int r = totS - preS - nS;
            const int lo = p0 > cut ? p0 : cut;
            for (int i = p1 - 1; i >= lo; i--)
                if (kd_less_w(a, a.kv[i], pk)) kd_swap(a, i, (int)box[r++]);
        }
        __builtin_amdgcn_wave_barrier();
        if (cut <= nth) first = cut; else last = cut;
    }
    kd_nth_element_team<64, 4>(a, first, nth, last, true, mb, depth);
}
#endif

OCTA_HD inline unsigned f32_bits(float v) { unsigned u; memcpy(&u, &v, 4); return u; }
OCTA_HD inline unsigned f32_sortable(float v) {
    unsigned u;
    memcpy(&u, &v, 4);
    return (u >> 31) ? ~u : (u | 0x80000000u);
}
OCTA_HD inline float f32_unsortable(unsigned e) {
    unsigned u = (e >> 31) ? (e & 0x7fffffffu) : ~e;
    float v;
    memcpy(&v, &u, 4);
    return v;
}
OCTA_HD inline float f32_round_up(double x) {
#if defined(__HIP_DEVICE_COMPILE__)
    return __double2float_ru(x);
#else
    float f = (float)x;
    return (double)f < x ? nextafterf(f, INFINITY) : f;
#endif
}
OCTA_HD inline float f32_round_down(double x) {
#if defined(__HIP_DEVICE_COMPILE__)
    return __double2float_rd(x);
#else
    float f = (float)x;
    return (double)f > x ? nextafterf(f, -INFINITY) : f;
#endif
}
OCTA_HD inline double f32_ulp(float v) {
    const float a = fabsf(v);
    return (double)nextafterf(a, INFINITY) - (double)a;
}
OCTA_HD inline void atomic_max_u32(unsigned *p, unsigned v) {
#if defined(__HIP_DEVICE_COMPILE__)
    atomicMax(p, v);
#else
    if (v > *p) *p = v;
#endif
}
OCTA_HD inline void atomic_min_u32(unsigned *p, unsigned v) {
#if defined(__HIP_DEVICE_COMPILE__)
    atomicMin(p, v);
#else
    if (v < *p) *p = v;
#endif
}

constexpr int KD_TAB_OFF = OCAP * (int)sizeof(kdw_t);
constexpr int KD_BOX_BYTES = KD_RANGES * 24;
static_assert(KD_RANGES >= OCAP / 17 + 1, "ranges per level");
static_assert(KD_MAILBOX_OFF % 16 == 0 && KD_MAILBOX_OFF >= KD_TAB_OFF + KD_RANGES * KD_TAB_BYTES_PER_RANGE, "kd tables overlap the mailbox");
static_assert(KD_MAILBOX_OFF + (KD_BOX_BYTES > KD_MAILBOX_BYTES ? KD_BOX_BYTES : KD_MAILBOX_BYTES) <= SIM_USER_BYTES, "kd table layout (box table and mailbox share their area)");
OCTA_HD inline void kd_build(const Blk &b, const double *pts, int n, idx_t *out_idx, idx_t *out_rank,
                              float *xy, double zlo, double zhi, long *kdprof = nullptr, const unsigned char *need = nullptr,
                              const bool flag_in_sign = false) {
#if defined(__HIP_DEVICE_COMPILE__) && !defined(OCTA_SIM_PROF_ASSIGN) && !defined(OCTA_SIM_PROF_SAMPLE) && !defined(OCTA_SIM_PROF_SET) && !defined(OCTA_SIM_PROF_MAIL) && !defined(OCTA_SIM_PROF_SEQ) && !defined(OCTA_SIM_PROF_SEQ2)
#define KDP(slot) do { if (kdprof && b.tid == 0) { long _t = (long)wall_clock64(); kdprof[slot] += _t - _kt; _kt = _t; } } while (0)
    long _kt = (long)wall_clock64();
#else
#define KDP(slot) do { } while (0)
#endif
    kdw_t *kv = reinterpret_cast<kdw_t *>(b.user_of<1>());
    idx_t *tab = reinterpret_cast<idx_t *>(b.user_of<1>() + KD_TAB_OFF);
    idx_t *rs = tab, *re = tab + KD_RANGES;
    idx_t *rs2 = tab + 2 * KD_RANGES, *re2 = tab + 3 * KD_RANGES;
    signed char *rd = reinterpret_cast<signed char *>(tab + 4 * KD_RANGES);
    unsigned *bbf = reinterpret_cast<unsigned *>(b.user_of<1>() + KD_MAILBOX_OFF);
#if defined(__HIP_DEVICE_COMPILE__) && !OCTA_SIM_LARGE
    if ((size_t)n * (sizeof(kdw_t) + 8) + 8 <= (size_t)KD_TAB_OFF)
        xy = reinterpret_cast<float *>(b.user_of<1>() + (((size_t)n * sizeof(kdw_t) + 7) & ~(size_t)7));
#endif
    for (int i = b.tid; i < n; i += b.nth) {
        kv[i] = (kdw_t)i;
        const float fx = (float)pts[3 * i];
        xy[2 * i] = (flag_in_sign && need[i]) ? -fx : fx; xy[2 * i + 1] = (float)pts[3 * i + 1];
    }
    if (b.tid == 0) { rs[0] = 0; re[0] = (idx_t)n; }
    const float z_up = f32_round_up(zhi), z_dn = f32_round_down(zlo);
    b.sync();
    int nr = (n > 16) ? 1 : 0;
    while (nr > 0) {
        for (int q = b.tid; q < nr; q += b.nth) {
            for (int k = 0; k < 2; k++) { bbf[6 * q + k] = 0u; bbf[6 * q + 3 + k] = ~0u; }
            bbf[6 * q + 2] = f32_sortable(z_up); bbf[6 * q + 5] = f32_sortable(z_dn);
            rd[q] = 0;
        }
        b.sync();
        {
            const int chunk = ((n + b.nth - 1) / b.nth) | 1;
            const int i0 = b.tid * chunk, i1 = (i0 + chunk < n) ? i0 + chunk : n;
            int q = 0;
            if (i0 < i1) {
                int lo_ = 0, hi_ = nr - 1;
                while (lo_ < hi_) { int mid = (lo_ + hi_ + 1) >> 1; if (rs[mid] <= i0) lo_ = mid; else hi_ = mid - 1; }
                q = lo_;
            }
            bool have = false, hit = false;
            float mx[2] = {0, 0}, mn[2] = {0, 0};
            auto flush = [&](int qq) {
                for (int k = 0; k < 2; k++) {
                    atomic_max_u32(&bbf[6 * qq + k], f32_sortable(nextafterf(mx[k], INFINITY)));
                    atomic_min_u32(&bbf[6 * qq + 3 + k], f32_sortable(nextafterf(mn[k], -INFINITY)));
                }
            };
            constexpr int KB = 8;
            int qw = q, cs = 0, ce = 0, ns = 0x7fffffff;
            if (i0 < i1) { cs = rs[qw]; ce = re[qw]; ns = qw + 1 < nr ? (int)rs[qw + 1] : 0x7fffffff; }
            for (int ib = i0; ib < i1; ib += KB) {
                int eq[KB], eid[KB];
                kdw_t ew[KB];
#pragma unroll
                for (int k = 0; k < KB; k++) ew[k] = kv[ib + k < i1 ? ib + k : i1 - 1];
#pragma unroll
                for (int k = 0; k < KB; k++) {
                    const int i = ib + k;
                    eq[k] = -1; eid[k] = 0;
                    if (i < i1) {
                        while (i >= ns) { qw++; cs = ns; ce = re[qw]; ns = qw + 1 < nr ? (int)rs[qw + 1] : 0x7fffffff; }
                        if (i >= cs && i < ce) { eq[k] = qw; eid[k] = (int)(ew[k] & KD_IDX_MASK); }
                    }
                }
                float ex[KB], ey[KB];
                unsigned char nd[KB];
#pragma unroll
                for (int k = 0; k < KB; k++) {
                    const float sx = xy[2 * eid[k]];
                    ex[k] = flag_in_sign ? fabsf(sx) : sx; ey[k] = xy[2 * eid[k] + 1];
                    nd[k] = flag_in_sign ? (unsigned char)(f32_bits(sx) >> 31) : (need ? need[eid[k]] : (unsigned char)1);
                }
#pragma unroll
                for (int k = 0; k < KB; k++) {
                    if (eq[k] < 0) continue;
                    if (eq[k] != q) {
                        if (have) { flush(q); have = false; }
                        if (hit) { rd[q] = 1; hit = false; }
                        q = eq[k];
                    }
                    if (nd[k]) hit = true;
                    if (!have) { mx[0] = mn[0] = ex[k]; mx[1] = mn[1] = ey[k]; }
                    else {
                        mx[0] = mx[0] > ex[k] ? mx[0] : ex[k]; mn[0] = mn[0] < ex[k] ? mn[0] : ex[k];
                        mx[1] = mx[1] > ey[k] ? mx[1] : ey[k]; mn[1] = mn[1] < ey[k] ? mn[1] : ey[k];
                    }
                    have = true;
                }
            }
            if (have) flush(q);
            if (hit) rd[q] = 1;
        }
        int *pend_n = b.coll() + 396, *pend = b.coll() + 420;
        if (b.tid == 0) *pend_n = 0;
        b.sync();
        KDP(0);
        for (int q = b.tid; q < nr; q += b.nth) {
            if (rd[q] == 0) { rd[q] = -1; continue; }
            double shi[3], slo[3];
            for (int k = 0; k < 3; k++) {
                const float up = f32_unsortable(bbf[6 * q + k]), dn = f32_unsortable(bbf[6 * q + 3 + k]);
                shi[k] = (double)up - (double)dn;
                slo[k] = shi[k] - 2.0 * (f32_ulp(up) + f32_ulp(dn));
            }
            slo[2] = 0.0;
            int d = 0;
            if (shi[1] > shi[d]) d = 1;
            if (shi[2] > shi[d]) d = 2;
            bool sure = true;
            for (int k = 0; k < 3; k++) if (k != d && !(slo[d] > shi[k])) sure = false;
            if (!OCTA_UNLIKELY(!sure)) { rd[q] = (signed char)d; continue; }
            if ((int)re[q] - (int)rs[q] > 256) {
                const int slot = atomic_add_int(pend_n, 1);
                if (slot < 64) { pend[slot] = q; rd[q] = (signed char)-2; continue; }
            }
            double hi3[3] = {0, 0, 0}, lo3[3] = {0, 0, 0};
            for (int i = rs[q]; i < re[q]; i++) {
                const double *p = pts + 3 * (int)(kv[i] & KD_IDX_MASK);
                for (int k = 0; k < 3; k++) {
                    if (i == rs[q]) { hi3[k] = lo3[k] = p[k]; }
                    else { hi3[k] = hi3[k] > p[k] ? hi3[k] : p[k]; lo3[k] = lo3[k] < p[k] ? lo3[k] : p[k]; }
                }
            }
            d = 0;
            double size = 0;
            for (int k = 0; k < 3; k++) if (hi3[k] - lo3[k] > size) { d = k; size = hi3[k] - lo3[k]; }
            rd[q] = (hi3[d] == lo3[d]) ? (signed char)-1 : (signed char)d;
        }
        b.sync();
        {
            const int n_pend = OCTA_UNI(*pend_n) < 64 ? OCTA_UNI(*pend_n) : 64;
            unsigned long long *ex = reinterpret_cast<unsigned long long *>(b.coll() + 400);
            for (int t = 0; t < n_pend; t++) {
                const int q = OCTA_UNI(pend[t]);
                for (int k = b.tid; k < 6; k += b.nth) ex[k] = k < 3 ? 0ull : ~0ull;
                b.sync();
                double hi3[3] = {0, 0, 0}, lo3[3] = {0, 0, 0};
                bool any = false;
                for (int i = (int)rs[q] + b.tid; i < (int)re[q]; i += b.nth) {
                    const double *p = pts + 3 * (int)(kv[i] & KD_IDX_MASK);
                    for (int k = 0; k < 3; k++) {
                        if (!any) { hi3[k] = lo3[k] = p[k]; }
                        else { hi3[k] = hi3[k] > p[k] ? hi3[k] : p[k]; lo3[k] = lo3[k] < p[k] ? lo3[k] : p[k]; }
                    }
                    any = true;
                }
                if (any)
                    for (int k = 0; k < 3; k++) { atomic_max_u64(&ex[k], dbl_sortable(hi3[k])); atomic_min_u64(&ex[3 + k], dbl_sortable(lo3[k])); }
                b.sync();
                if (b.tid == 0) {
                    int d = 0;
                    double size = 0, lo_d = 0, hi_d = 0;
                    for (int k = 0; k < 3; k++) {
                        const double hk = dbl_unsortable(ex[k]), lk = dbl_unsortable(ex[3 + k]);
                        if (k == 0) { hi_d = hk; lo_d = lk; }
                        if (hk - lk > size) { d = k; size = hk - lk; hi_d = hk; lo_d = lk; }
                    }
                    rd[q] = (hi_d == lo_d) ? (signed char)-1 : (signed char)d;
                }
                b.sync();
            }
        }
        KDP(1);
        {
            const int chunk = ((n + b.nth - 1) / b.nth) | 1;
            const int i0 = b.tid * chunk, i1 = (i0 + chunk < n) ? i0 + chunk : n;
            int q = 0;
            if (i0 < i1) {
                int lo_ = 0, hi_ = nr - 1;
                while (lo_ < hi_) { int mid = (lo_ + hi_ + 1) >> 1; if (rs[mid] <= i0) lo_ = mid; else hi_ = mid - 1; }
                q = lo_;
            }
            int qc = -1, d = -1;
            double mnd = 0, scale = 0;
            int cs = 0, ce = 0, ns = 0x7fffffff;
            if (i0 < i1) { cs = rs[q]; ce = re[q]; ns = q + 1 < nr ? (int)rs[q + 1] : 0x7fffffff; }
            for (int i = i0; i < i1; i++) {
                while (i >= ns) { q++; cs = ns; ce = re[q]; ns = q + 1 < nr ? (int)rs[q + 1] : 0x7fffffff; }
                if (i < cs || i >= ce) continue;
                if (q != qc) {
                    qc = q; d = rd[q];
                    if (d >= 0) {
                        mnd = (double)f32_unsortable(bbf[6 * q + 3 + d]);
                        const double w = (double)f32_unsortable(bbf[6 * q + d]) - mnd;
                        scale = w > 0.0 ? (double)KD_QMAX / w : 0.0;
                    }
                }
                if (d >= 0) {
                    const unsigned id = (unsigned)(kv[i] & KD_IDX_MASK);
                    const float fv = d < 2 ? xy[2 * id + d] : 0.f;
                    const double cv = d < 2 ? (double)((flag_in_sign && d == 0) ? fabsf(fv) : fv) : pts[3 * id + 2];
                    kv[i] = (kd_quant(cv, mnd, scale) << KD_IDX_BITS) | (kdw_t)id;
                }
            }
        }
        b.sync();
        KDP(2);
#if defined(__HIP_DEVICE_COMPILE__)
        {
            idx_t *mb = reinterpret_cast<idx_t *>(b.user_of<1>() + KD_MAILBOX_OFF);
            const int wv = b.tid >> 6, nw = (b.nth + 63) >> 6;
            for (int q = wv; q < nr; q += nw) {
                int d = rd[q];
                int s = rs[q], e = re[q];
                if (d < 0 || e - s < KD_TEAM_MIN) continue;
                const KdPair kp = {kv, pts, d};
                if (e - s > KD_MASK_MAX) kd_nth_element_wave_long(kp, s, s + (e - s) / 2, e, mb);
                else if (e - s > 4000) kd_nth_element_team<64, 4>(kp, s, s + (e - s) / 2, e, true, mb);
                else kd_nth_element_team<64, 1>(kp, s, s + (e - s) / 2, e, true, mb);
            }
        }
        KDP(3);
        {
            idx_t *mb = reinterpret_cast<idx_t *>(b.user_of<1>() + KD_MAILBOX_OFF);
            const int team = b.tid >> 4, nteam = b.nth >> 4;
            for (int q0 = 0; q0 < nr; q0 += nteam) {
                int q = q0 + team;
                bool live = q < nr;
                int s = 0, e = 0, d = 0;
                if (live) {
                    s = rs[q]; e = re[q]; d = rd[q];
                    live = d >= 0 && e - s < KD_TEAM_MIN;
                }
                const KdPair kp = {kv, pts, d < 0 ? 0 : d};
                kd_nth_element_team<16, 1>(kp, s, s + (e - s) / 2, e, live, mb);
            }
        }
#else
        for (int q = b.tid; q < nr; q += b.nth) {
            int d = rd[q];
            if (d < 0) continue;
            int s = rs[q], e = re[q];
            const KdPair kp = {kv, pts, d};
            kd_nth_element(kp, s, s + (e - s) / 2, e);
        }
#endif
        b.sync();
        KDP(4);
        {
            int base = 0;
            for (int q0 = 0; q0 < nr; q0 += b.nth) {
                const int q = q0 + b.tid;
                int s = 0, e = 0, m = 0, c = 0;
                if (q < nr && rd[q] >= 0) {
                    s = rs[q]; e = re[q]; m = s + (e - s) / 2;
                    c = (m - s > 16 ? 1 : 0) + (e - m > 16 ? 1 : 0);
                }
                int ex;
                const int tot = blk_scan(b, c, &ex);
                int pos = base + ex;
                if (m - s > 16) { if (pos < KD_RANGES) { rs2[pos] = (idx_t)s; re2[pos] = (idx_t)m; } pos++; }
                if (e - m > 16) { if (pos < KD_RANGES) { rs2[pos] = (idx_t)m; re2[pos] = (idx_t)e; } }
                base += tot;
            }
            nr = base < KD_RANGES ? base : KD_RANGES;
        }
        { idx_t *t = rs; rs = rs2; rs2 = t; t = re; re = re2; re2 = t; }
        KDP(5);
    }
    for (int i = b.tid; i < n; i += b.nth) { const idx_t id = (idx_t)(kv[i] & KD_IDX_MASK); out_idx[i] = id; out_rank[id] = (idx_t)i; }
    b.sync();
    KDP(6);
#undef KDP
}


constexpr int GRID_N = NCAP > OCAP ? NCAP : OCAP;
struct Grid {
    int nx, ny;
    double x0, y0, inv, cell;
    const int *cell_end;
    const idx_t *items;
    const double *spts;
    const float *sptf;
    const double *src;
};
OCTA_HD inline int grid_clampi(int v, int hi) { return v < 0 ? 0 : (v > hi ? hi : v); }
OCTA_HD inline int grid_cx(const Grid &G, double x) { return grid_clampi((int)floor((x - G.x0) * G.inv), G.nx - 1); }
OCTA_HD inline int grid_cy(const Grid &G, double y) { return grid_clampi((int)floor((y - G.y0) * G.inv), G.ny - 1); }

OCTA_HD inline Grid grid_build_once(const Blk &b, const SimArrays &A, const double *pts, const int *ids, int n, double radius, int div, bool as_float,
                                    const unsigned char *mask) {
    Grid G;
    const double span = 1.2;
    double cell = fmax(radius / div, span / GRID_MAX);
    int nc = (int)ceil(span / cell);
    if (nc < 1) nc = 1;
    if (nc > GRID_MAX) nc = GRID_MAX;
    G.nx = G.ny = nc; G.x0 = G.y0 = -0.1; G.inv = 1.0 / cell; G.cell = cell;
    const int ncell = nc * nc;
    int *hist = reinterpret_cast<int *>(b.user_of<2>());
    idx_t *items = reinterpret_cast<idx_t *>(b.user_of<2>() + (size_t)(GRID_MAX * GRID_MAX + 1) * 4);
    static_assert((size_t)(GRID_MAX * GRID_MAX + 1) * 4 + (size_t)GRID_N * sizeof(idx_t) <= (size_t)SIM_USER_BYTES, "grid table layout");
    G.cell_end = hist; G.items = items; G.spts = A.grid_pts; G.sptf = reinterpret_cast<const float *>(A.grid_pts); G.src = pts;
    if (n > GRID_N) n = GRID_N;
    b.sync();
    for (int c = b.tid; c <= ncell; c += b.nth) hist[c] = 0;
    b.sync();
    constexpr int GB = 4;
    for (int i0 = b.tid; i0 < n; i0 += GB * b.nth) {
        double px[GB], py[GB];
        bool live[GB];
#pragma unroll
        for (int k = 0; k < GB; k++) {
            const int i = i0 + k * b.nth;
            const int ic = i < n ? i : n - 1;
            const double *p = pts + 3 * (ids ? ids[ic] : ic);
            px[k] = p[0]; py[k] = p[1];
            live[k] = i < n && (!mask || mask[ic]);
        }
#pragma unroll
        for (int k = 0; k < GB; k++)
            if (live[k]) atomic_add_int(&hist[grid_cy(G, py[k]) * nc + grid_cx(G, px[k])], 1);
    }
    b.sync();
    {
        const int total = ncell + 1;
        const int chunk = ((total + b.nth - 1) / b.nth) | 1;
        const int c0 = b.tid * chunk, c1 = (c0 + chunk < total) ? c0 + chunk : total;
        int local = 0;
        for (int c = c0; c < c1; c++) local += hist[c];
        int ex;
        blk_scan(b, local, &ex);
        int run = ex;
        for (int c = c0; c < c1; c++) { int v = hist[c]; hist[c] = run; run += v; }
    }
    b.sync();
    for (int i0 = b.tid; i0 < n; i0 += GB * b.nth) {
        V3 p[GB];
        int id[GB];
        bool live[GB];
#pragma unroll
        for (int k = 0; k < GB; k++) {
            const int i = i0 + k * b.nth;
            const int ic = i < n ? i : n - 1;
            id[k] = ids ? ids[ic] : ic;
            p[k] = ld3(pts + 3 * id[k]);
            live[k] = i < n && (!mask || mask[ic]);
        }
#pragma unroll
        for (int k = 0; k < GB; k++)
            if (live[k]) {
                int pos = atomic_add_int(&hist[grid_cy(G, p[k].y) * nc + grid_cx(G, p[k].x)], 1);
                items[pos] = (idx_t)id[k];
                if (as_float) { float *f = reinterpret_cast<float *>(A.grid_pts) + 3 * pos; f[0] = (float)p[k].x; f[1] = (float)p[k].y; f[2] = (float)p[k].z; }
                else st3(A.grid_pts + 3 * pos, p[k]);
            }
    }
    b.sync();
    return G;
}
OCTA_HD inline Grid grid_build(const Blk &b, const SimArrays &A, const double *pts, const int *ids, int n, double radius, int div = 1,
                               bool as_float = false, const unsigned char *mask = nullptr) {
#if OCTA_SIM_DUP & 2
    grid_build_once(b, A, pts, ids, n, radius, div, as_float, mask);
#endif
    return grid_build_once(b, A, pts, ids, n, radius, div, as_float, mask);
}
constexpr int GRID_VB = 4;
constexpr double GRID_F_TAU = 1e-6;
struct Pt3f { float x, y, z; };
OCTA_HD inline float sqdist_f(Pt3f a, float cx, float cy, float cz) { const float dx = a.x - cx, dy = a.y - cy, dz = a.z - cz; return fmaf(dz, dz, fmaf(dy, dy, dx * dx)); }
template <bool FLT> struct GridPt;
template <> struct GridPt<false> { typedef V3 T; static OCTA_HD inline V3 load(const Grid &G, int k) { return ld3(G.spts + 3 * k); } static OCTA_HD inline V3 zero() { return v3(0, 0, 0); } };
template <> struct GridPt<true> {
    typedef Pt3f T;
    static OCTA_HD inline Pt3f load(const Grid &G, int k) { const float *f = G.sptf + 3 * k; Pt3f r = {f[0], f[1], f[2]}; return r; }
    static OCTA_HD inline Pt3f zero() { Pt3f r = {0.f, 0.f, 0.f}; return r; }
};
template <bool FLT, class F>
OCTA_HD inline void grid_visit_impl(const Grid &G, double px, double py, double radius, F &&body) {
    const int cy0 = grid_cy(G, py - radius), cy1 = grid_cy(G, py + radius);
    const int cx0 = grid_cx(G, px - radius), cx1 = grid_cx(G, px + radius);
    for (int cyb = cy0; cyb <= cy1; cyb += 3) {
        int k0[3], k1[3];
#pragma unroll
        for (int r = 0; r < 3; r++) {
            const int row = cyb + r;
            k0[r] = k1[r] = 0;
            if (row <= cy1) {
                const int c0 = row * G.nx + cx0;
                k0[r] = c0 ? G.cell_end[c0 - 1] : 0;
                k1[r] = G.cell_end[row * G.nx + cx1];
            }
        }
        typename GridPt<FLT>::T pt[3][GRID_VB];
        int it[3][GRID_VB];
#pragma unroll
        for (int r = 0; r < 3; r++)
#pragma unroll
            for (int u = 0; u < GRID_VB; u++) {
                const int k = k0[r] + u < k1[r] ? k0[r] + u : k0[r];
                pt[r][u] = k0[r] < k1[r] ? GridPt<FLT>::load(G, k) : GridPt<FLT>::zero();
                it[r][u] = k0[r] < k1[r] ? (int)G.items[k] : 0;
            }
#pragma unroll
        for (int r = 0; r < 3; r++) {
#pragma unroll
            for (int u = 0; u < GRID_VB; u++)
// ... 1608 lines not shown
            if (b.tid == 128) sc->flush_rounds += rounds;
        }
    }
#else
    (void)side; (void)side_lds;
#endif
#undef SEQT
#undef SEQ2_TOP
#undef SEQ2_SEL
#undef SEQ2_END
#undef SEQ2_ARG
    b.sync();
#if defined(__HIP_DEVICE_COMPILE__)
    if (b.tid == 0 && pend_other > 0) sc->fl_pending[1 - f] = 0;
#endif
    {
        long t0 = OCTA_FLUSH_T0();
        const int rounds = murray_flush(b, A, f, L, b.coll()[91]);
        if (b.tid == 0) {
            sc->kdprof[7] += OCTA_FLUSH_T0() - t0; sc->flush_rounds += rounds;
#if defined(OCTA_SIM_PROF_SEQ) && defined(__HIP_DEVICE_COMPILE__)
            sc->kdprof[3] += OCTA_FLUSH_T0() - t0;
#endif
        }
    }
    b.sync();
}

OCTA_HD inline void murray_flush_pending(const Blk &b, const SimArrays &A) {
#if defined(__HIP_DEVICE_COMPILE__)
    b.sync();
    double *fl_val = reinterpret_cast<double *>(b.user_of<8>());
    int *fl_done = reinterpret_cast<int *>(fl_val + MURRAY_FLUSH_LDS);
    for (int f = 0; f < 2; f++) {
        const int n = OCTA_UNI(A.sc->fl_pending[f]);
        if (n <= 0) continue;
        for (int i = b.tid; i < MURRAY_FLUSH_LDS / 32; i += b.nth) fl_done[i] = 0;
        b.sync();
        const int wv = b.tid >> 6;
        if (wv < 3 && wv * 64 < n) {
            const int rounds = murray_flush_rounds_wave(A.nrad_of(f), octa_gpow::LOG_TAB, octa_gpow::EXP_TAB, fl_val, fl_done, A.fl_rec + (size_t)f * MURRAY_FLUSH_LDS, n,
                                                        wv, 3, true);
            if (b.tid == 0) { A.sc->fl_pending[f] = 0; A.sc->flush_rounds += rounds; }
        }
        b.sync();
    }
#else
    (void)b; (void)A;
#endif
}

constexpr int COMPACT_TILE = 3072;
constexpr int COMPACT_TILE_NN = 2048;
OCTA_HD inline int compact_points(const Blk &b, double *pts, int n, const unsigned char *removed, double *stage, int *c_nn = nullptr,
                                  double *c_d2 = nullptr) {
    (void)stage;
    if (b.nth == 1) {
        int w = 0;
        for (int i = 0; i < n; i++)
            if (!removed[i]) {
                if (w != i) {
                    pts[3 * w] = pts[3 * i]; pts[3 * w + 1] = pts[3 * i + 1]; pts[3 * w + 2] = pts[3 * i + 2];
                    if (c_nn) { c_nn[w] = c_nn[i]; c_d2[w] = c_d2[i]; }
                }
                w++;
            }
        return w;
    }
    double *tile = reinterpret_cast<double *>(b.user_of<16>());
    static_assert((size_t)COMPACT_TILE * 24 <= (size_t)SIM_USER_BYTES && (size_t)COMPACT_TILE_NN * 36 <= (size_t)SIM_USER_BYTES, "compaction tile");
#if defined(__HIP_DEVICE_COMPILE__)
    const int lane = b.tid & 63, wv = b.tid >> 6, nw = (b.nth + 63) >> 6;
    const int TILE = c_nn ? COMPACT_TILE_NN : COMPACT_TILE;
    double *td = tile + 3 * COMPACT_TILE_NN;
    int *ti = reinterpret_cast<int *>(td + COMPACT_TILE_NN);
    int base = 0;
    for (int t0 = 0; t0 < n; t0 += TILE) {
        const int tn = n - t0 < TILE ? n - t0 : TILE;
        const int seg = ((tn + nw * 64 - 1) / (nw * 64)) * 64;
        const int s0 = t0 + (wv * seg < tn ? wv * seg : tn), s1 = s0 + seg < t0 + tn ? s0 + seg : t0 + tn;
        int c = 0;
        for (int i0 = s0; i0 < s1; i0 += 64) c += (int)__popcll(__ballot(i0 + lane < s1 && !removed[i0 + lane]));
        int ex;
        const int kept = blk_scan(b, lane == 0 ? c : 0, &ex);
        if (base != t0 || kept != tn) {
            int at = __builtin_amdgcn_readfirstlane(ex);
            constexpr int CB = 2;
            for (int i0 = s0; i0 < s1; i0 += CB * 64) {
                bool keep[CB];
                V3 v[CB];
                int vn[CB] = {};
                double vd[CB] = {};
#pragma unroll
                for (int u = 0; u < CB; u++) {
                    const int i = i0 + u * 64 + lane, ic = i < s1 ? i : s1 - 1;
                    keep[u] = i < s1 && !removed[ic];
                    v[u] = ld3(pts + 3 * (size_t)ic);
                    if (c_nn) { vn[u] = c_nn[ic]; vd[u] = c_d2[ic]; }
                }
                OCTA_ISSUE_LOADS();
#pragma unroll
                for (int u = 0; u < CB; u++) {
                    const unsigned long long m = __ballot(keep[u]);
                    if (keep[u]) {
                        const int w = at + (int)__popcll(m & ((1ull << lane) - 1ull));
                        tile[3 * w] = v[u].x; tile[3 * w + 1] = v[u].y; tile[3 * w + 2] = v[u].z;
                        if (c_nn) { ti[w] = vn[u]; td[w] = vd[u]; }
                    }
                    at += (int)__popcll(m);
                }
            }
            b.sync();
            for (int j = b.tid; j < kept * 3; j += b.nth) pts[(size_t)3 * base + j] = tile[j];
            if (c_nn)
                for (int j = b.tid; j < kept; j += b.nth) { c_nn[base + j] = ti[j]; c_d2[base + j] = td[j]; }
            b.sync();
        }
        base += kept;
    }
    return base;
#else
    (void)tile;
    return n;
#endif
}

OCTA_HD inline bool assign_memory_covers(const SimArrays &A, int f, int n) {
#ifdef OCTA_SIM_ASSIGN_NOCACHE
    (void)A; (void)f; (void)n;
    return false;
#else
    return OCTA_UNI((int)(A.nn_prev_of(f) != nullptr && A.sc->n_cached[f] == n)) != 0;
#endif
}

#if defined(__HIP_DEVICE_COMPILE__)
#define OCTA_SUBPROF(sc, slot, t0) do { if (b.tid == 0) { long _t1 = (long)wall_clock64(); (sc)->prof[slot] += _t1 - (t0); (t0) = _t1; } } while (0)
#define OCTA_SUBPROF_T0() ((long)wall_clock64())
#else
#define OCTA_SUBPROF(sc, slot, t0) do { (void)(t0); } while (0)
#define OCTA_SUBPROF_T0() 0L
#endif

OCTA_HD inline void phase_satisfy_art(const Blk &b, const SimArrays &A, const SimConst &C, const IterParams &P) {
    const double zext = C.sz;
    SampleScalars *sc = A.sc;
    const int nb = sc->new_begin[0], ne = sc->new_end[0];
    const int n_new = ne - nb, n_oxy = sc->n_oxy;
    if (n_new <= 0 || n_oxy <= 0) return;
    const double ek = P.eps_k, ek2 = ek * ek;
    long t0 = OCTA_SUBPROF_T0();
    for (int i = b.tid; i < n_oxy; i += b.nth) A.removed[i] = 0;
    int *ctl = b.coll() + 100;
    if (b.tid == 0) { ctl[0] = 0; ctl[1] = 0; }
    b.sync();
    {
        int *new_ids = A.tmp_int;
        for (int j = b.tid; j < n_new; j += b.nth) new_ids[j] = nb + j;
        b.sync();
        Grid G = grid_build(b, A, A.npos[0], new_ids, n_new, ek);
        for (int o = b.tid; o < n_oxy; o += b.nth) {
            const V3 p = ld3(A.oxy + 3 * o);
            grid_visit(G, p.x, p.y, ek, [&](int j, const V3 &q) {
                if (sqdist(p, q) <= ek2) {
                    int slot = atomic_add_int(&ctl[0], 1);
                    if (slot < PCAP) A.pairs[slot] = ((unsigned)(j - nb) << IDX_BITS) | (unsigned)o;
                    A.removed[o] = 1;
                }
            });
        }
        b.sync();
    }
    OCTA_SUBPROF(sc, 12, t0);
    int n_pairs = ctl[0];
    if (n_pairs > PCAP) { if (b.tid == 0) atomic_or_int(&sc->err, ERR_PAIR_CAP); n_pairs = PCAP; }
    if (n_new > (1 << (32 - IDX_BITS))) { if (b.tid == 0) atomic_or_int(&sc->err, ERR_PAIR_CAP); }
    b.sync();
    if (n_pairs == 0) return;
    {
        const int n_ven = sc->n_nodes[1];
        int *rem = A.tmp_int;
        int n_rem = 0;
        {
            const int chunk = (n_oxy + b.nth - 1) / b.nth;
            const int i0 = b.tid * chunk < n_oxy ? b.tid * chunk : n_oxy, i1 = (i0 + chunk < n_oxy) ? i0 + chunk : n_oxy;
            int local = 0;
            for (int o = i0; o < i1; o++) local += A.removed[o] ? 1 : 0;
            int ex;
            n_rem = blk_scan(b, local, &ex);
            int run = ex;
            for (int o = i0; o < i1; o++) if (A.removed[o]) rem[run++] = o;
        }
        b.sync();
        for (int k = b.tid; k < n_rem; k += b.nth) {
            const int o = rem[k];
            A.ven_near[o] = 0;
            A.hashes[o] = py_hash_tuple3(ld3(A.oxy + 3 * o));
        }
        Grid G = grid_build(b, A, A.oxy, rem, n_rem, ek);
        constexpr int VB = 4;
        for (int j0 = b.tid; j0 < n_ven; j0 += VB * b.nth) {
            V3 qv[VB];
#pragma unroll
            for (int u = 0; u < VB; u++) { const int j = j0 + u * b.nth; qv[u] = ld3(A.npos[1] + 3 * (j < n_ven ? j : n_ven - 1)); }
#pragma unroll
            for (int u = 0; u < VB; u++) {
                if (j0 + u * b.nth >= n_ven) break;
                const V3 q = qv[u];
                grid_visit(G, q.x, q.y, ek, [&](int o, const V3 &p) {
                    if (sqrt(sqdist(q, p)) <= ek) A.ven_near[o] = 1;
                });
            }
        }
        b.sync();
    }
    OCTA_SUBPROF(sc, 12, t0);
    bool set_in_lds = false, ranked = false;
#ifdef OCTA_SIM_DEBUG_SAT
    int dbg_n_ins = -1, dbg_mask = -1, dbg_base = -1;
    const int dbg_n_co2_in = sc->n_co2;
#endif
    for (int pass = 0; pass < 2; pass++) {
        ranked = pass > 0;
        if (ranked) {
            kd_build(b, A.oxy, n_oxy, A.kd_idx, A.kd_rank, reinterpret_cast<float *>(A.tmp_dbl), 0.0, zext, sc->kdprof, A.removed, true);
#if OCTA_SIM_DUP & 1
            kd_build(b, A.oxy, n_oxy, A.kd_idx, A.kd_rank, reinterpret_cast<float *>(A.tmp_dbl), 0.0, zext, nullptr, A.removed, true);
#endif
            for (int i = b.tid; i < n_pairs; i += b.nth) {
                unsigned pr = A.pairs[i];
                A.pairs[i] = (pr & ~IDX_MASK) | (unsigned)A.kd_rank[pr & IDX_MASK];
            }
            b.sync();
            OCTA_SUBPROF(sc, 11, t0);
        }
        unsigned *keys = reinterpret_cast<unsigned *>(b.user_of<32>());
        int n_pow2 = 1;
        while (n_pow2 < n_pairs) n_pow2 <<= 1;
        for (int i = b.tid; i < n_pow2; i += b.nth) keys[i] = i < n_pairs ? A.pairs[i] : 0xffffffffu;
        b.sync();
        if (n_pairs > 0) blk_sort_u32(b, keys, n_pow2);
        for (int i = b.tid; i < n_pairs; i += b.nth) A.pairs[i] = keys[i];
        b.sync();
        OCTA_SUBPROF(sc, 13, t0);
#if defined(__HIP_DEVICE_COMPILE__)
#if defined(OCTA_SIM_PROF_SET)
        long _pt = (long)wall_clock64();
#define PSP(slot) do { if (b.tid == 0) { long _t = (long)wall_clock64(); sc->kdprof[slot] += _t - _pt; _pt = _t; } } while (0)
#else
#define PSP(slot) do { } while (0)
#endif
        constexpr int EMPTY = 0x7fffffff;
        auto replay = [&](int *own, int *in_key, unsigned long long *in_hash, int *dk, unsigned long long *dh, int *ord0, int *ord1,
                          const int s_max) __attribute__((always_inline)) -> int {
            int n_ins = 0;
            for (int p0 = 0; p0 < n_pairs; p0 += b.nth) {
                const int i = p0 + b.tid;
                int o = -1, take = 0;
                unsigned long long hsh = 0;
                if (i < n_pairs) {
                    o = ranked ? (int)A.kd_idx[keys[i] & IDX_MASK] : (int)(keys[i] & IDX_MASK);
                    take = A.ven_near[o] ? 0 : 1;
                    hsh = A.hashes[o];
                }
                int ex;
                const int tot = blk_scan(b, take, &ex);
                if (take) { in_key[n_ins + ex] = (int)((keys[i] & ~IDX_MASK) | (unsigned)o); in_hash[n_ins + ex] = hsh; }
                n_ins += tot;
            }
            b.sync();
            PSP(0);
            for (int i = b.tid; i < n_ins; i += b.nth) own[(unsigned)in_key[i] & IDX_MASK] = EMPTY;
            b.sync();
            for (int i = b.tid; i < n_ins; i += b.nth) atomic_min_int(&own[(unsigned)in_key[i] & IDX_MASK], i);
            b.sync();
            int D = 0;
            for (int p0 = 0; p0 < n_ins; p0 += b.nth) {
                const int i = p0 + b.tid;
                const bool first = i < n_ins && own[(unsigned)in_key[i] & IDX_MASK] == i;
                int ex;
                const int tot = blk_scan(b, first ? 1 : 0, &ex);
                if (first) { dk[D + ex] = in_key[i]; dh[D + ex] = in_hash[i]; }
                D += tot;
            }
            b.sync();
            PSP(1);
            int S = 8, n_prev = 0;
            int *ord = ord0, *ord_next = ord1;
            while (true) {
                const int thr = (3 * (S - 1) + 4) / 5;
                const int upto = D < thr ? D : thr;
                const unsigned long long mask = (unsigned long long)(S - 1);
                for (int p = n_prev + b.tid; p < upto; p += b.nth) ord[p] = p;
                for (int e = b.tid; e < S; e += b.nth) own[e] = EMPTY;
                b.sync();
                for (int p = b.tid; p < upto; p += b.nth) {
                    int cur = p;
                    unsigned long long hsh = dh[ord[cur]], i = hsh & mask, perturb = hsh;
                    int lin = 0, nlin = (i + 9 <= mask) ? 9 : 0;
                    auto next = [&] {
                        if (lin < nlin) { lin++; return; }
                        perturb >>= 5;
                        i = (i * 5 + 1 + perturb) & mask;
                        nlin = (i + 9 <= mask) ? 9 : 0; lin = 0;
                    };
                    while (true) {
                        const int slot = (int)i + lin;
                        const int old = atomic_min_ret_int(&own[slot], cur);
                        if (old == EMPTY) break;
                        if (old > cur) {
                            cur = old;
                            hsh = dh[ord[cur]]; i = hsh & mask; perturb = hsh; lin = 0; nlin = (i + 9 <= mask) ? 9 : 0;
                            while ((int)i + lin != slot) next();
                        }
                        next();
                    }
                }
                b.sync();
                if (!ranked) {
                    for (int p = n_prev + b.tid; p < upto; p += b.nth) {
                        const unsigned g = (unsigned)dk[p] >> IDX_BITS;
                        const unsigned long long hsh = dh[p];
                        unsigned long long i = hsh & mask, perturb = hsh;
                        int lin = 0, nlin = (i + 9 <= mask) ? 9 : 0;
                        while (true) {
                            const int q = own[(int)i + lin];
                            if (q == p) break;
                            if (q == EMPTY) { atomic_or_int(&ctl[1], 1); break; }
                            if (q >= n_prev && ((unsigned)dk[q] >> IDX_BITS) == g) { atomic_or_int(&ctl[1], 1); break; }
                            if (lin < nlin) { lin++; continue; }
                            perturb >>= 5;
                            i = (i * 5 + 1 + perturb) & mask;
                            nlin = (i + 9 <= mask) ? 9 : 0; lin = 0;
                        }
                    }
                    if (b.tid == 0 && D > thr && ((unsigned)dk[thr - 1] >> IDX_BITS) == ((unsigned)dk[thr] >> IDX_BITS)) atomic_or_int(&ctl[1], 1);
                    b.sync();
                    if (ctl[1]) break;
                }
                if (D < thr) break;
                const int minused = upto > 50000 ? upto * 2 : upto * 4;
                int newS = 8;
                while (newS <= minused) newS <<= 1;
                if (newS > s_max) { if (b.tid == 0) atomic_or_int(&sc->err, ERR_SET_CAP); break; }
                {
                    const int lane = b.tid & 63, wv = b.tid >> 6, nw = (b.nth + 63) >> 6;
                    const int seg = ((S + nw * 64 - 1) / (nw * 64)) * 64;
                    const int s0 = wv * seg < S ? wv * seg : S, s1 = s0 + seg < S ? s0 + seg : S;
                    int c = 0;
                    for (int e0 = s0; e0 < s1; e0 += 64) c += (int)__popcll(__ballot(e0 + lane < s1 && own[e0 + lane] != EMPTY));
                    int ex;
                    blk_scan(b, lane == 0 ? c : 0, &ex);
                    int at = __builtin_amdgcn_readfirstlane(ex);
                    for (int e0 = s0; e0 < s1; e0 += 64) {
                        const int pr = e0 + lane < s1 ? own[e0 + lane] : EMPTY;
                        const unsigned long long m = __ballot(pr != EMPTY);
                        if (pr != EMPTY) ord_next[at + (int)__popcll(m & ((1ull << lane) - 1ull))] = ord[pr];
                        at += (int)__popcll(m);
                    }
                }
                b.sync();
                { int *t = ord; ord = ord_next; ord_next = t; }
                n_prev = upto;
                S = newS;
            }
            PSP(2);
            for (int e = b.tid; e < S; e += b.nth) { const int pr = own[e]; own[e] = pr == EMPTY ? -1 : (int)((unsigned)dk[ord[pr]] & IDX_MASK); }
            b.sync();
            PSP(3);
#ifdef OCTA_SIM_DEBUG_SAT
            dbg_n_ins = n_ins;
#endif
            return S - 1;
        };
        constexpr bool HBM_REPLAY = (size_t)PCAP + OCAP <= (size_t)OCAP + 2 * (size_t)NCANDCAP && (size_t)OCAP * 2 <= (size_t)OCAP * 3
                                    && PCAP <= SETCAP && OCAP <= SETCAP;
        const int *t_key = nullptr;
        int mask = -1;
        if (n_pairs <= LSET_PAIRS) {
            constexpr int S_MAX = LSET_CAP / 2;
            int *own = reinterpret_cast<int *>(b.user_of<64>());
            constexpr int OWN_N = OCAP > S_MAX ? OCAP : S_MAX;
            int *in_key = own + OWN_N;
            int *dk = in_key + LSET_PAIRS, *ord0 = dk + LSET_PAIRS, *ord1 = ord0 + LSET_PAIRS;
            unsigned long long *in_hash = reinterpret_cast<unsigned long long *>(ord1 + LSET_PAIRS + ((OWN_N + 4 * LSET_PAIRS) & 1));
            unsigned long long *dh = in_hash + LSET_PAIRS;
            static_assert((size_t)(OWN_N + 4 * LSET_PAIRS + 1) * 4 + (size_t)2 * LSET_PAIRS * 8 <= (size_t)SIM_USER_BYTES, "set replay layout");
            static_assert((size_t)LSET_PAIRS * 4 <= (size_t)OWN_N * 4, "the sorted pairs (start of the table area) end before the insert stream");
            mask = replay(own, in_key, in_hash, dk, dh, ord0, ord1, S_MAX);
            t_key = own;
            set_in_lds = true;
        } else if (HBM_REPLAY && n_pairs <= PCAP) {
            int *own = A.set_key;
            int *in_key = A.tmp_int, *ord0 = A.tmp_int + PCAP;
            unsigned long long *in_hash = A.set_hash;
            unsigned long long *dh = reinterpret_cast<unsigned long long *>(A.tmp_dbl);
            int *dk = reinterpret_cast<int *>(A.tmp_dbl + OCAP), *ord1 = dk + OCAP;
            mask = replay(own, in_key, in_hash, dk, dh, ord0, ord1, SETCAP / 2);
            t_key = own;
            set_in_lds = true;
        }
        if (set_in_lds && (ranked || !ctl[1])) {
            const int n_co2_0 = sc->n_co2;
            int base = 0;
            {
                const int per = (mask + 1 + b.nth - 1) / b.nth;
                const int e0 = b.tid * per < mask + 1 ? b.tid * per : mask + 1, e1 = e0 + per < mask + 1 ? e0 + per : mask + 1;
                int cnt = 0;
                for (int e = e0; e < e1; e++) cnt += t_key[e] >= 0 ? 1 : 0;
                int ex2;
                base = blk_scan(b, cnt, &ex2);
                int dst = n_co2_0 + ex2;
                constexpr int RB = 8;
                for (int eb = e0; eb < e1; eb += RB) {
                    int k[RB];
                    V3 v[RB];
#pragma unroll
                    for (int u = 0; u < RB; u++) { k[u] = eb + u < e1 ? t_key[eb + u] : -1; }
#pragma unroll
                    for (int u = 0; u < RB; u++) v[u] = ld3(A.oxy + 3 * (k[u] >= 0 ? k[u] : 0));
#pragma unroll
                    for (int u = 0; u < RB; u++)
                        if (k[u] >= 0) { if (dst < CCAP) st3(A.co2 + 3 * dst, v[u]); dst++; }
                }
            }
            b.sync();
            PSP(4);
            if (b.tid == 0) {
                int n_co2 = n_co2_0 + base;
                if (n_co2 > CCAP) { sc->err |= ERR_CO2_CAP; n_co2 = CCAP; }
                sc->n_co2 = n_co2;
            }
#ifdef OCTA_SIM_DEBUG_SAT
            dbg_mask = mask; dbg_base = base;
#endif
        }
#undef PSP
#endif
        if (!set_in_lds && b.tid == 0) {
            PySetView S;
            S.hash = A.set_hash; S.key = A.set_key; S.err = &sc->err; S.cap = SETCAP;
            pyset_init(S);
            int *cw = reinterpret_cast<int *>(A.tmp_dbl);
            static_assert((size_t)SETCAP / 2 <= (size_t)2 * OCAP, "certificate table");
            int D = 0;
            for (int i = 0; i < n_pairs; i++) {
                const unsigned pr = A.pairs[i];
                const int o = ranked ? (int)A.kd_idx[pr & IDX_MASK] : (int)(pr & IDX_MASK);
                if (!A.ven_near[o]) {
                    const int used = S.used;
                    pyset_add(S, o, A.hashes[o]);
                    if (!ranked && S.used != used) { cw[D] = o; cw[OCAP + D] = (int)(pr >> IDX_BITS); D++; }
                }
            }
            if (!ranked && !pyset_order_free(cw, cw + OCAP, A.hashes, D, cw + 4 * OCAP, cw + 2 * OCAP, cw + 3 * OCAP, SETCAP / 2)) ctl[1] = 1;
            if (ranked || !ctl[1]) {
                int n_co2 = sc->n_co2;
                for (int e = 0; e <= S.mask; e++)
                    if (S.key[e] >= 0) {
                        if (n_co2 >= CCAP) { sc->err |= ERR_CO2_CAP; break; }
                        int o = S.key[e];
                        A.co2[3 * n_co2] = A.oxy[3 * o]; A.co2[3 * n_co2 + 1] = A.oxy[3 * o + 1]; A.co2[3 * n_co2 + 2] = A.oxy[3 * o + 2];
                        n_co2++;
                    }
                sc->n_co2 = n_co2;
            }
        }
        b.sync();
        OCTA_SUBPROF(sc, 14, t0);
        if (!ranked && ctl[1]) continue;
        if (b.tid == 0) sc->kd_path[ranked ? 1 : 0]++;
        break;
    }
#if defined(OCTA_SIM_DEBUG_SAT) && !defined(OCTA_SIM_ITER_PROF)
    {
        int ex, loc;
        loc = 0; for (int o = b.tid; o < n_oxy; o += b.nth) loc += A.removed[o] ? 1 : 0;
        const int c_rem = blk_scan(b, loc, &ex);
        loc = 0; for (int o = b.tid; o < n_oxy; o += b.nth) loc += (A.removed[o] && A.ven_near[o]) ? 1 : 0;
        const int c_ven = blk_scan(b, loc, &ex);
        unsigned char *mark = reinterpret_cast<unsigned char *>(A.tmp_dbl);
        for (int o = b.tid; o < 2 * n_oxy; o += b.nth) mark[o] = 0;
        b.sync();
        for (int i = b.tid; i < n_pairs; i += b.nth) {
            const int o = ranked ? (int)A.kd_idx[A.pairs[i] & IDX_MASK] : (int)(A.pairs[i] & IDX_MASK);
            mark[o] = 1;
            if (!A.ven_near[o]) mark[n_oxy + o] = 1;
        }
        b.sync();
        loc = 0; for (int o = b.tid; o < n_oxy; o += b.nth) loc += mark[o];
        const int c_pair_all = blk_scan(b, loc, &ex);
        loc = 0; for (int o = b.tid; o < n_oxy; o += b.nth) loc += mark[n_oxy + o];
        const int c_pair_take = blk_scan(b, loc, &ex);
        loc = 0; for (int o = b.tid; o < n_oxy; o += b.nth) loc += (mark[o] != (A.removed[o] ? 1 : 0)) ? 1 : 0;
        const int c_pair_vs_removed = blk_scan(b, loc, &ex);
        int c_slots = -1, c_in_distinct = -1, c_slot_bad = -1;
        if (set_in_lds) {
            const int *t_key = reinterpret_cast<const int *>(b.user());
            const int *in_key = t_key + (OCAP > LSET_CAP / 2 ? OCAP : LSET_CAP / 2);
            loc = 0; for (int e = b.tid; e <= dbg_mask; e += b.nth) loc += t_key[e] >= 0 ? 1 : 0;
            c_slots = blk_scan(b, loc, &ex);
            loc = 0; for (int e = b.tid; e <= dbg_mask; e += b.nth) { const int k = t_key[e]; if (k >= 0 && (k >= n_oxy || !A.removed[k] || A.ven_near[k])) loc++; }
            c_slot_bad = blk_scan(b, loc, &ex);
            for (int o = b.tid; o < n_oxy; o += b.nth) mark[o] = 0;
            b.sync();
            for (int i = b.tid; i < dbg_n_ins; i += b.nth) { const int k = (int)((unsigned)in_key[i] & IDX_MASK); if (k < n_oxy) mark[k] = 1; }
            b.sync();
            loc = 0; for (int o = b.tid; o < n_oxy; o += b.nth) loc += mark[o];
            c_in_distinct = blk_scan(b, loc, &ex);
        }
        b.sync();
        if (b.tid == 0 && A.dbg) {
            int *row = A.dbg + 16 * A.dbg_it;
            row[0] = n_new; row[1] = n_oxy; row[2] = n_pairs; row[3] = c_rem; row[4] = c_ven; row[5] = c_pair_all; row[6] = c_pair_take;
            row[7] = c_pair_vs_removed; row[8] = dbg_n_ins; row[9] = dbg_mask; row[10] = dbg_base; row[11] = c_slots; row[12] = c_in_distinct;
            row[13] = c_slot_bad; row[14] = dbg_n_co2_in; row[15] = sc->n_co2;
        }
        b.sync();
    }
#endif
    const bool carry = assign_memory_covers(A, 0, n_oxy);
    int keep = compact_points(b, A.oxy, n_oxy, A.removed, A.tmp_dbl, carry ? A.nn_prev[0] : nullptr, carry ? A.nn_d2[0] : nullptr);
    if (b.tid == 0) { sc->n_oxy = keep; sc->n_cached[0] = carry ? keep : 0; }
    b.sync();
    OCTA_SUBPROF(sc, 15, t0);
}

OCTA_HD inline void phase_satisfy_ven(const Blk &b, const SimArrays &A, const IterParams &P) {
    SampleScalars *sc = A.sc;
    const int nb = sc->new_begin[1], ne = sc->new_end[1];
    const int n_new = ne - nb, n_co2 = sc->n_co2;
    if (n_new <= 0 || n_co2 <= 0) return;
    const double ek2 = P.eps_k * P.eps_k;
    const double ek = P.eps_k;
    {
        int *new_ids = A.tmp_int;
        for (int j = b.tid; j < n_new; j += b.nth) new_ids[j] = nb + j;
        b.sync();
        Grid G = grid_build(b, A, A.npos[1], new_ids, n_new, ek);
        for (int o = b.tid; o < n_co2; o += b.nth) {
            const V3 p = ld3(A.co2 + 3 * o);
            bool hit = false;
            grid_visit(G, p.x, p.y, ek, [&](int, const V3 &q) {
                if (!hit && sqdist(p, q) <= ek2) hit = true;
            });
            A.removed[o] = hit ? 1 : 0;
        }
        b.sync();
    }
    const bool carry = assign_memory_covers(A, 1, n_co2);
    int keep = compact_points(b, A.co2, n_co2, A.removed, A.tmp_dbl, carry ? A.nn_prev[1] : nullptr, carry ? A.nn_d2[1] : nullptr);
    if (b.tid == 0) { sc->n_co2 = keep; sc->n_cached[1] = carry ? keep : 0; }
    b.sync();
}

}
```

Baseline: 1448.

## Add partial kd-ranking rung and sparse live-range kd build passes

Replaces the two-pass (unranked, then fully ranked) set-ordering fallback with a three-rung ladder. The middle rung re-ranks only the groups flagged as violating the Python set order, tracking those groups with per-group flags. Separately, kd_build now tracks how many points are still live and, when few remain, iterates only over live ranges instead of all n points. Both aim to cut redundant full kd work in the sink-assignment step. The cost is more complex control flow and an extra rung that may fail and fall through to the full rebuild.

```diff
diff --git a/include/octa_hip.h b/include/octa_hip.h
--- a/include/octa_hip.h
+++ b/include/octa_hip.h
@@ -305,6 +305,8 @@
 
 int octa_sim_kat_kd_order(octa_ctx *ctx, const double *h_pts, int64_t n, const uint8_t *h_need, int32_t *h_indices);
 
+int octa_sim_kat_kd_order_signflag(octa_ctx *ctx, const double *h_pts, int64_t n, const uint8_t *h_need, int32_t need_bits, int32_t *h_indices);
+
 #ifdef __cplusplus
 }
 #endif
diff --git a/octa_autosegmentation_amd/_native.py b/octa_autosegmentation_amd/_native.py
--- a/octa_autosegmentation_amd/_native.py
+++ b/octa_autosegmentation_amd/_native.py
@@ -143,6 +143,7 @@
     "octa_frangi_hessian": (c_int, [c_void_p, c_void_p, c_void_p, c_void_p, c_int, c_int, c_int, c_int, c_void_p, ctypes.c_float, c_int, c_void_p, c_void_p]),
     "octa_frangi_eigenvalues": (c_int, [c_void_p, c_void_p, c_void_p, c_void_p, c_int, c_int, c_int, c_int, c_void_p, ctypes.c_float, c_int, c_void_p, c_void_p]),
     "octa_sim_kat_kd_order": (c_int, [c_void_p, c_void_p, ctypes.c_int64, c_void_p, c_void_p]),
+    "octa_sim_kat_kd_order_signflag": (c_int, [c_void_p, c_void_p, ctypes.c_int64, c_void_p, ctypes.c_int32, c_void_p]),
 }
 
 
diff --git a/octa_autosegmentation_amd/csrc/sim.hip b/octa_autosegmentation_amd/csrc/sim.hip
--- a/octa_autosegmentation_amd/csrc/sim.hip
+++ b/octa_autosegmentation_amd/csrc/sim.hip
@@ -36,6 +36,7 @@
 #define octa_sim_spans OCTA_SIM_FN(spans)
 #define octa_sim_timing OCTA_SIM_FN(timing)
 #define octa_sim_kat_kd_order OCTA_SIM_FN(kat_kd_order)
+#define octa_sim_kat_kd_order_signflag OCTA_SIM_FN(kat_kd_order_signflag)
 struct OCTA_SIM_T;
 extern "C" void octa_sim_destroy(OCTA_SIM_T *S);
 extern "C" long long octa_sim_next_ticket(void);
@@ -1284,7 +1285,8 @@
 
 extern "C" int octa_sim_kd_paths(OCTA_SIM_T *S, int64_t *h_paths) {
     if (!S || !S->ran || !h_paths) { octa::set_error("octa_sim_kd_paths: run the simulation first"); return -2; }
-    for (int s = 0; s < S->B; s++) { h_paths[2 * s] = S->h_sc[s].kd_path[0]; h_paths[2 * s + 1] = S->h_sc[s].kd_path[1]; }
+    for (int s = 0; s < S->B; s++)
+        for (int k = 0; k < 3; k++) h_paths[3 * s + k] = S->h_sc[s].kd_path[k];
     return 0;
 }
 
@@ -1315,15 +1317,30 @@
 #if !OCTA_SIM_LARGE
 namespace {
 __global__ void __launch_bounds__(SIM_THREADS)
-sim_kat_kd_kernel(const double *pts, int n, const unsigned char *need, idx_t *out_idx, idx_t *out_rank, float *xy, double zlo, double zhi) {
+sim_kat_kd_kernel(const double *pts, int n, const unsigned char *need, idx_t *out_idx, idx_t *out_rank, float *xy, double zlo, double zhi,
+                  int flag_in_sign, int need_bits) {
     extern __shared__ __attribute__((aligned(16))) unsigned char smem[];
     Blk b = {(int)threadIdx.x, (int)blockDim.x, smem};
-    kd_build(b, pts, n, out_idx, out_rank, xy, zlo, zhi, nullptr, need);
-}
+    kd_build(b, pts, n, out_idx, out_rank, xy, zlo, zhi, nullptr, need, flag_in_sign != 0, (unsigned char)need_bits);
+}
+
+int kat_kd_order(octa_ctx *ctx, const double *h_pts, int64_t n, const uint8_t *h_need, int32_t *h_indices, int flag_in_sign, int need_bits);
 }
 
 extern "C" int octa_sim_kat_kd_order(octa_ctx *ctx, const double *h_pts, int64_t n, const uint8_t *h_need, int32_t *h_indices) {
     if (!ctx || !h_pts || !h_indices || n < 0 || n > OCAP) { octa::set_error("octa_sim_kat_kd_order: bad arguments"); return -2; }
+    return kat_kd_order(ctx, h_pts, n, h_need, h_indices, 0, 0xff);
+}
+
+extern "C" int octa_sim_kat_kd_order_signflag(octa_ctx *ctx, const double *h_pts, int64_t n, const uint8_t *h_need, int32_t need_bits, int32_t *h_indices) {
+    if (!ctx || !h_pts || !h_need || !h_indices || n < 0 || n > OCAP || need_bits <= 0 || need_bits > 0xff) { octa::set_error("octa_sim_kat_kd_order_signflag: bad arguments"); return -2; }
+    for (int64_t i = 0; i < n; i++)
+        if (!(h_pts[3 * i] >= 0.0)) { octa::set_error("octa_sim_kat_kd_order_signflag: x must be >= 0"); return -2; }
+    return kat_kd_order(ctx, h_pts, n, h_need, h_indices, 1, need_bits);
+}
+
+namespace {
+int kat_kd_order(octa_ctx *ctx, const double *h_pts, int64_t n, const uint8_t *h_need, int32_t *h_indices, int flag_in_sign, int need_bits) {
     if (n == 0) return 0;
     OCTA_HIP_CHECK(hipSetDevice(ctx->device));
     double *d_pts = nullptr;
@@ -1341,7 +1358,7 @@
         OCTA_HIP_CHECK(hipMemcpy(d_need, h_need, n, hipMemcpyHostToDevice));
     }
     OCTA_HIP_CHECK(hipFuncSetAttribute(reinterpret_cast<const void *>(sim_kat_kd_kernel), hipFuncAttributeMaxDynamicSharedMemorySize, (int)SIM_LDS));
-    hipLaunchKernelGGL(sim_kat_kd_kernel, dim3(1), dim3(SIM_THREADS), SIM_LDS, 0, d_pts, (int)n, d_need, d_idx, d_idx + n, d_xy, zlo, zhi);
+    hipLaunchKernelGGL(sim_kat_kd_kernel, dim3(1), dim3(SIM_THREADS), SIM_LDS, 0, d_pts, (int)n, d_need, d_idx, d_idx + n, d_xy, zlo, zhi, flag_in_sign, need_bits);
     OCTA_HIP_CHECK(hipGetLastError());
     std::vector<idx_t> h(n);
     OCTA_HIP_CHECK(hipMemcpy(h.data(), d_idx, sizeof(idx_t) * n, hipMemcpyDeviceToHost));
@@ -1349,6 +1366,7 @@
     (void)hipFree(d_pts); (void)hipFree(d_idx); (void)hipFree(d_xy); if (d_need) (void)hipFree(d_need);
     return 0;
 }
+}
 
 #endif
 
diff --git a/octa_autosegmentation_amd/csrc/sim_api.cpp b/octa_autosegmentation_amd/csrc/sim_api.cpp
--- a/octa_autosegmentation_amd/csrc/sim_api.cpp
+++ b/octa_autosegmentation_amd/csrc/sim_api.cpp
@@ -29,6 +29,7 @@
 OCTA_DECL(L, octa_simL_impl)
 #undef OCTA_DECL
 int octa_simS_kat_kd_order(octa_ctx *, const double *, int64_t, const uint8_t *, int32_t *);
+int octa_simS_kat_kd_order_signflag(octa_ctx *, const double *, int64_t, const uint8_t *, int32_t, int32_t *);
 }
 
 #include <atomic>
@@ -116,4 +117,5 @@
 }
 extern "C" int octa_sim_geometry(int num_cus, int *h_out4) { return octa_simS_geometry(num_cus, h_out4); }
 extern "C" int octa_sim_kat_kd_order(octa_ctx *ctx, const double *p, int64_t n, const uint8_t *need, int32_t *o) { return octa_simS_kat_kd_order(ctx, p, n, need, o); }
+extern "C" int octa_sim_kat_kd_order_signflag(octa_ctx *ctx, const double *p, int64_t n, const uint8_t *need, int32_t bits, int32_t *o) { return octa_simS_kat_kd_order_signflag(ctx, p, n, need, bits, o); }
 extern "C" int octa_sim_is_large(const octa_sim *sim) { return sim && sim->large ? 1 : 0; }
diff --git a/octa_autosegmentation_amd/csrc/sim_core.h b/octa_autosegmentation_amd/csrc/sim_core.h
--- a/octa_autosegmentation_amd/csrc/sim_core.h
+++ b/octa_autosegmentation_amd/csrc/sim_core.h
@@ -61,6 +61,16 @@
 constexpr int KD_TAB_BYTES_PER_RANGE = 4 * (int)sizeof(idx_t) + 1;
 constexpr int KD_MAILBOX_OFF = OCAP * (int)sizeof(kdw_t) + ((KD_RANGES * KD_TAB_BYTES_PER_RANGE + 15) / 16) * 16;
 constexpr int KD_TEAM_MIN = 192;
+#ifndef OCTA_SIM_KD_SPARSE
+#define OCTA_SIM_KD_SPARSE 8192
+#endif
+constexpr int KD_SPARSE_MAX = OCTA_SIM_KD_SPARSE, KD_SPARSE_RANGES = 32;
+constexpr int KD_COLL_PEND_N = 396;
+constexpr int KD_COLL_LIVE_N = 397;
+constexpr int KD_COLL_EXTREMA = 400;
+constexpr int KD_COLL_PEND = 420;
+static_assert(KD_COLL_PEND_N >= 384 && KD_COLL_LIVE_N == KD_COLL_PEND_N + 1 && KD_COLL_EXTREMA % 2 == 0 && KD_COLL_EXTREMA > KD_COLL_LIVE_N &&
+              KD_COLL_PEND >= KD_COLL_EXTREMA + 12 && (KD_COLL_PEND + 64) * 4 <= 2048, "kd_build's collective words");
 #ifndef OCTA_SIM_THREADS
 #define OCTA_SIM_THREADS 256
 #endif
@@ -127,7 +137,7 @@
     long respec;
     long prof[16];
     long kdprof[8];
-    int kd_path[2];
+    int kd_path[3];
     int resume_it, resume_stage;
     int parked, finished;
     long t_begin, t_end;
@@ -555,9 +565,9 @@
     }
 }
 
-OCTA_HD inline bool pyset_order_free(const int *dk, const int *dg, const unsigned long long *hashes, int D, int *own, int *ord0, int *ord1,
-                                     int s_max) {
-    int S = 8, n_prev = 0;
+OCTA_HD inline int pyset_order_check(const int *dk, const int *dg, const unsigned long long *hashes, int D, int *own, int *ord0, int *ord1,
+                                     int s_max, unsigned char *xf, bool second) {
+    int S = 8, n_prev = 0, viol = 0;
     int *ord = ord0, *ord_next = ord1;
     while (true) {
         const int thr = (3 * (S - 1) + 4) / 5;
@@ -569,6 +579,7 @@
             const int k = ord[p];
             const unsigned long long hsh = hashes[dk[k]];
             unsigned long long perturb = hsh, i = hsh & mask;
+            bool check = p >= n_prev && !(second && xf[dg[k]]);
             while (true) {
                 unsigned long long e = i;
                 int probes = (i + 9 <= mask) ? 9 : 0;
@@ -576,7 +587,10 @@
                 do {
                     const int q = own[e];
                     if (q < 0) { own[e] = p; placed = true; break; }
-                    if (p >= n_prev && q >= n_prev && dg[q] == dg[k]) return false;
+                    if (check && q >= n_prev && dg[q] == dg[k]) {
+                        if (!xf || second) return 1;
+                        xf[dg[k]] = 1; viol++; check = false;
+                    }
                     e++;
                 } while (probes--);
                 if (placed) break;
@@ -584,18 +598,26 @@
                 i = (i * 5 + 1 + perturb) & mask;
             }
         }
-        if (D < thr) return true;
-        if (D > thr && dg[thr - 1] == dg[thr]) return false;
+        if (D < thr) return viol;
+        if (D > thr && dg[thr - 1] == dg[thr]) {
+            if (!xf) return 1;
+            if (!second) { xf[dg[thr]] = 1; viol++; }
+            else if (!xf[dg[thr]]) return 1;
+        }
         const int minused = upto > 50000 ? upto * 2 : upto * 4;
         int newS = 8;
         while (newS <= minused) newS <<= 1;
-        if (newS > s_max) return false;
+        if (newS > s_max) return 1;
         int c = 0;
         for (int e = 0; e < S; e++) if (own[e] >= 0) ord_next[c++] = ord[own[e]];
         { int *t = ord; ord = ord_next; ord_next = t; }
         n_prev = upto;
         S = newS;
     }
+}
+OCTA_HD inline bool pyset_order_free(const int *dk, const int *dg, const unsigned long long *hashes, int D, int *own, int *ord0, int *ord1,
+                                     int s_max) {
+    return pyset_order_check(dk, dg, hashes, D, own, ord0, ord1, s_max, nullptr, false) == 0;
 }
 
 constexpr int KD_IDX_BITS = IDX_BITS;
@@ -934,7 +956,7 @@
 static_assert(KD_MAILBOX_OFF + (KD_BOX_BYTES > KD_MAILBOX_BYTES ? KD_BOX_BYTES : KD_MAILBOX_BYTES) <= SIM_USER_BYTES, "kd table layout (box table and mailbox share their area)");
 OCTA_HD inline void kd_build(const Blk &b, const double *pts, int n, idx_t *out_idx, idx_t *out_rank,
                               float *xy, double zlo, double zhi, long *kdprof = nullptr, const unsigned char *need = nullptr,
-                              const bool flag_in_sign = false) {
+                              const bool flag_in_sign = false, const unsigned char need_bits = 0xff) {
 #if defined(__HIP_DEVICE_COMPILE__) && !defined(OCTA_SIM_PROF_ASSIGN) && !defined(OCTA_SIM_PROF_SAMPLE) && !defined(OCTA_SIM_PROF_SET) && !defined(OCTA_SIM_PROF_MAIL) && !defined(OCTA_SIM_PROF_SEQ) && !defined(OCTA_SIM_PROF_SEQ2)
 #define KDP(slot) do { if (kdprof && b.tid == 0) { long _t = (long)wall_clock64(); kdprof[slot] += _t - _kt; _kt = _t; } } while (0)
     long _kt = (long)wall_clock64();
@@ -954,9 +976,10 @@
     for (int i = b.tid; i < n; i += b.nth) {
         kv[i] = (kdw_t)i;
         const float fx = (float)pts[3 * i];
-        xy[2 * i] = (flag_in_sign && need[i]) ? -fx : fx; xy[2 * i + 1] = (float)pts[3 * i + 1];
-    }
-    if (b.tid == 0) { rs[0] = 0; re[0] = (idx_t)n; }
+        xy[2 * i] = (flag_in_sign && (need[i] & need_bits)) ? -fx : fx; xy[2 * i + 1] = (float)pts[3 * i + 1];
+    }
+    int *live_n = b.coll() + KD_COLL_LIVE_N;
+    if (b.tid == 0) { rs[0] = 0; re[0] = (idx_t)n; *live_n = n; }
     const float z_up = f32_round_up(zhi), z_dn = f32_round_down(zlo);
     b.sync();
     int nr = (n > 16) ? 1 : 0;
@@ -967,14 +990,21 @@
             rd[q] = 0;
         }
         b.sync();
+        const int live = OCTA_UNI(*live_n);
+        const bool sparse = live <= KD_SPARSE_MAX && 2 * live <= n && nr <= KD_SPARSE_RANGES;
+        const int span = sparse ? live : n;
         {
-            const int chunk = ((n + b.nth - 1) / b.nth) | 1;
-            const int i0 = b.tid * chunk, i1 = (i0 + chunk < n) ? i0 + chunk : n;
-            int q = 0;
-            if (i0 < i1) {
+            const int chunk = ((span + b.nth - 1) / b.nth) | 1;
+            const int i0 = b.tid * chunk, i1 = (i0 + chunk < span) ? i0 + chunk : span;
+            int q = 0, vs = 0, ve = 0;
+            if (i0 < i1 && !sparse) {
                 int lo_ = 0, hi_ = nr - 1;
                 while (lo_ < hi_) { int mid = (lo_ + hi_ + 1) >> 1; if (rs[mid] <= i0) lo_ = mid; else hi_ = mid - 1; }
                 q = lo_;
+            }
+            if (i0 < i1 && sparse) {
+                ve = (int)re[0] - (int)rs[0];
+                while (i0 >= ve && q + 1 < nr) { q++; vs = ve; ve = vs + (int)re[q] - (int)rs[q]; }
             }
             bool have = false, hit = false;
             float mx[2] = {0, 0}, mn[2] = {0, 0};
@@ -990,15 +1020,30 @@
             for (int ib = i0; ib < i1; ib += KB) {
                 int eq[KB], eid[KB];
                 kdw_t ew[KB];
-#pragma unroll
-                for (int k = 0; k < KB; k++) ew[k] = kv[ib + k < i1 ? ib + k : i1 - 1];
-#pragma unroll
-                for (int k = 0; k < KB; k++) {
-                    const int i = ib + k;
-                    eq[k] = -1; eid[k] = 0;
-                    if (i < i1) {
-                        while (i >= ns) { qw++; cs = ns; ce = re[qw]; ns = qw + 1 < nr ? (int)rs[qw + 1] : 0x7fffffff; }
-                        if (i >= cs && i < ce) { eq[k] = qw; eid[k] = (int)(ew[k] & KD_IDX_MASK); }
+                if (sparse) {
+#pragma unroll
+                    for (int k = 0; k < KB; k++) {
+                        const int i = ib + k;
+                        eq[k] = -1; eid[k] = 0;
+                        if (i < i1) {
+                            while (i >= ve && qw + 1 < nr) { qw++; cs = rs[qw]; ce = re[qw]; vs = ve; ve = vs + ce - cs; }
+                            const int at = cs + (i - vs);
+                            if (at < ce) { eq[k] = qw; eid[k] = at; }
+                        }
+                    }
+#pragma unroll
+                    for (int k = 0; k < KB; k++) eid[k] = (int)(kv[eid[k]] & KD_IDX_MASK);
+                } else {
+#pragma unroll
+                    for (int k = 0; k < KB; k++) ew[k] = kv[ib + k < i1 ? ib + k : i1 - 1];
+#pragma unroll
+                    for (int k = 0; k < KB; k++) {
+                        const int i = ib + k;
+                        eq[k] = -1; eid[k] = 0;
+                        if (i < i1) {
+                            while (i >= ns) { qw++; cs = ns; ce = re[qw]; ns = qw + 1 < nr ? (int)rs[qw + 1] : 0x7fffffff; }
+                            if (i >= cs && i < ce) { eq[k] = qw; eid[k] = (int)(ew[k] & KD_IDX_MASK); }
+                        }
                     }
                 }
                 float ex[KB], ey[KB];
@@ -1007,7 +1052,7 @@
                 for (int k = 0; k < KB; k++) {
                     const float sx = xy[2 * eid[k]];
                     ex[k] = flag_in_sign ? fabsf(sx) : sx; ey[k] = xy[2 * eid[k] + 1];
-                    nd[k] = flag_in_sign ? (unsigned char)(f32_bits(sx) >> 31) : (need ? need[eid[k]] : (unsigned char)1);
+                    nd[k] = flag_in_sign ? (unsigned char)(f32_bits(sx) >> 31) : (need ? (unsigned char)(need[eid[k]] & need_bits) : (unsigned char)1);
                 }
 #pragma unroll
                 for (int k = 0; k < KB; k++) {
@@ -1029,9 +1074,10 @@
             if (have) flush(q);
             if (hit) rd[q] = 1;
         }
-        int *pend_n = b.coll() + 396, *pend = b.coll() + 420;
+        int *pend_n = b.coll() + KD_COLL_PEND_N, *pend = b.coll() + KD_COLL_PEND;
         if (b.tid == 0) *pend_n = 0;
         b.sync();
+        if (b.tid == 0) *live_n = 0;
         KDP(0);
         for (int q = b.tid; q < nr; q += b.nth) {
             if (rd[q] == 0) { rd[q] = -1; continue; }
@@ -1068,7 +1114,7 @@
         b.sync();
         {
             const int n_pend = OCTA_UNI(*pend_n) < 64 ? OCTA_UNI(*pend_n) : 64;
-            unsigned long long *ex = reinterpret_cast<unsigned long long *>(b.coll() + 400);
+            unsigned long long *ex = reinterpret_cast<unsigned long long *>(b.coll() + KD_COLL_EXTREMA);
             for (int t = 0; t < n_pend; t++) {
                 const int q = OCTA_UNI(pend[t]);
                 for (int k = b.tid; k < 6; k += b.nth) ex[k] = k < 3 ? 0ull : ~0ull;
@@ -1101,21 +1147,32 @@
         }
         KDP(1);
         {
-            const int chunk = ((n + b.nth - 1) / b.nth) | 1;
-            const int i0 = b.tid * chunk, i1 = (i0 + chunk < n) ? i0 + chunk : n;
-            int q = 0;
-            if (i0 < i1) {
+            const int chunk = ((span + b.nth - 1) / b.nth) | 1;
+            const int i0 = b.tid * chunk, i1 = (i0 + chunk < span) ? i0 + chunk : span;
+            int q = 0, vs = 0, ve = 0;
+            if (i0 < i1 && !sparse) {
                 int lo_ = 0, hi_ = nr - 1;
                 while (lo_ < hi_) { int mid = (lo_ + hi_ + 1) >> 1; if (rs[mid] <= i0) lo_ = mid; else hi_ = mid - 1; }
                 q = lo_;
+            }
+            if (i0 < i1 && sparse) {
+                ve = (int)re[0] - (int)rs[0];
+                while (i0 >= ve && q + 1 < nr) { q++; vs = ve; ve = vs + (int)re[q] - (int)rs[q]; }
             }
             int qc = -1, d = -1;
             double mnd = 0, scale = 0;
             int cs = 0, ce = 0, ns = 0x7fffffff;
             if (i0 < i1) { cs = rs[q]; ce = re[q]; ns = q + 1 < nr ? (int)rs[q + 1] : 0x7fffffff; }
-            for (int i = i0; i < i1; i++) {
-                while (i >= ns) { q++; cs = ns; ce = re[q]; ns = q + 1 < nr ? (int)rs[q + 1] : 0x7fffffff; }
-                if (i < cs || i >= ce) continue;
+            for (int v = i0; v < i1; v++) {
+                int i = v;
+                if (sparse) {
+                    while (v >= ve && q + 1 < nr) { q++; cs = rs[q]; ce = re[q]; vs = ve; ve = vs + ce - cs; }
+                    i = cs + (v - vs);
+                    if (i >= ce) continue;
+                } else {
+                    while (i >= ns) { q++; cs = ns; ce = re[q]; ns = q + 1 < nr ? (int)rs[q + 1] : 0x7fffffff; }
+                    if (i < cs || i >= ce) continue;
+                }
                 if (q != qc) {
                     qc = q; d = rd[q];
                     if (d >= 0) {
@@ -1183,6 +1240,7 @@
                 if (q < nr && rd[q] >= 0) {
                     s = rs[q]; e = re[q]; m = s + (e - s) / 2;
                     c = (m - s > 16 ? 1 : 0) + (e - m > 16 ? 1 : 0);
+                    if (c) atomic_add_int(live_n, (m - s > 16 ? m - s : 0) + (e - m > 16 ? e - m : 0));
                 }
                 int ex;
                 const int tot = blk_scan(b, c, &ex);
@@ -3097,7 +3155,10 @@
     long t0 = OCTA_SUBPROF_T0();
     for (int i = b.tid; i < n_oxy; i += b.nth) A.removed[i] = 0;
     int *ctl = b.coll() + 100;
-    if (b.tid == 0) { ctl[0] = 0; ctl[1] = 0; }
+    if (b.tid == 0) { ctl[0] = 0; ctl[1] = 0; ctl[2] = 0; }
+    unsigned char *xf = reinterpret_cast<unsigned char *>(A.nn);
+    static_assert((size_t)NCAP <= (size_t)OCAP * sizeof(int), "group flags fit the nearest-node list");
+    for (int j = b.tid; j < n_new && j < NCAP; j += b.nth) xf[j] = 0;
     b.sync();
     {
         int *new_ids = A.tmp_int;
@@ -3160,21 +3221,40 @@
         b.sync();
     }
     OCTA_SUBPROF(sc, 12, t0);
-    bool set_in_lds = false, ranked = false;
+    bool set_in_lds = false;
+    int rung = 0;
+    bool from_partial = false;
+    auto sink_of = [&](unsigned pr) -> int {
+        const unsigned low = pr & IDX_MASK;
+        return (rung == 2 || (rung == 1 && xf[pr >> IDX_BITS])) ? (int)A.kd_idx[low] : (int)low;
+    };
 #ifdef OCTA_SIM_DEBUG_SAT
     int dbg_n_ins = -1, dbg_mask = -1, dbg_base = -1;
     const int dbg_n_co2_in = sc->n_co2;
 #endif
-    for (int pass = 0; pass < 2; pass++) {
-        ranked = pass > 0;
-        if (ranked) {
-            kd_build(b, A.oxy, n_oxy, A.kd_idx, A.kd_rank, reinterpret_cast<float *>(A.tmp_dbl), 0.0, zext, sc->kdprof, A.removed, true);
+    while (true) {
+        const int vslot = rung == 1 ? 2 : 1;
+        if (rung > 0) {
+            if (rung == 1) {
+                for (int i = b.tid; i < n_pairs; i += b.nth) {
+                    const unsigned pr = A.pairs[i];
+                    if (xf[pr >> IDX_BITS]) A.removed[pr & IDX_MASK] = 3;
+                }
+            } else if (OCTA_UNLIKELY(from_partial)) {
+                for (int i = b.tid; i < n_pairs; i += b.nth) {
+                    const unsigned pr = A.pairs[i];
+                    if (xf[pr >> IDX_BITS]) A.pairs[i] = (pr & ~IDX_MASK) | (unsigned)A.kd_idx[pr & IDX_MASK];
+                }
+            }
+            b.sync();
+            const unsigned char need_bits = rung == 1 ? (unsigned char)2 : (unsigned char)0xff;
+            kd_build(b, A.oxy, n_oxy, A.kd_idx, A.kd_rank, reinterpret_cast<float *>(A.tmp_dbl), 0.0, zext, sc->kdprof, A.removed, true, need_bits);
 #if OCTA_SIM_DUP & 1
-            kd_build(b, A.oxy, n_oxy, A.kd_idx, A.kd_rank, reinterpret_cast<float *>(A.tmp_dbl), 0.0, zext, nullptr, A.removed, true);
+            kd_build(b, A.oxy, n_oxy, A.kd_idx, A.kd_rank, reinterpret_cast<float *>(A.tmp_dbl), 0.0, zext, nullptr, A.removed, true, need_bits);
 #endif
             for (int i = b.tid; i < n_pairs; i += b.nth) {
                 unsigned pr = A.pairs[i];
-                A.pairs[i] = (pr & ~IDX_MASK) | (unsigned)A.kd_rank[pr & IDX_MASK];
+                if (rung == 2 || xf[pr >> IDX_BITS]) A.pairs[i] = (pr & ~IDX_MASK) | (unsigned)A.kd_rank[pr & IDX_MASK];
             }
             b.sync();
             OCTA_SUBPROF(sc, 11, t0);
@@ -3204,7 +3284,7 @@
                 int o = -1, take = 0;
                 unsigned long long hsh = 0;
                 if (i < n_pairs) {
-                    o = ranked ? (int)A.kd_idx[keys[i] & IDX_MASK] : (int)(keys[i] & IDX_MASK);
+                    o = sink_of(keys[i]);
                     take = A.ven_near[o] ? 0 : 1;
                     hsh = A.hashes[o];
                 }
@@ -3262,26 +3342,37 @@
                     }
                 }
                 b.sync();
-                if (!ranked) {
+                if (rung < 2) {
                     for (int p = n_prev + b.tid; p < upto; p += b.nth) {
                         const unsigned g = (unsigned)dk[p] >> IDX_BITS;
+                        if (rung == 1 && xf[g]) continue;
                         const unsigned long long hsh = dh[p];
                         unsigned long long i = hsh & mask, perturb = hsh;
                         int lin = 0, nlin = (i + 9 <= mask) ? 9 : 0;
                         while (true) {
                             const int q = own[(int)i + lin];
                             if (q == p) break;
-                            if (q == EMPTY) { atomic_or_int(&ctl[1], 1); break; }
-                            if (q >= n_prev && ((unsigned)dk[q] >> IDX_BITS) == g) { atomic_or_int(&ctl[1], 1); break; }
+                            if (q == EMPTY || (q >= n_prev && ((unsigned)dk[q] >> IDX_BITS) == g)) {
+                                if (rung == 0) xf[g] = 1;
+                                atomic_or_int(&ctl[vslot], 1);
+                                break;
+                            }
                             if (lin < nlin) { lin++; continue; }
                             perturb >>= 5;
                             i = (i * 5 + 1 + perturb) & mask;
                             nlin = (i + 9 <= mask) ? 9 : 0; lin = 0;
                         }
                     }
-                    if (b.tid == 0 && D > thr && ((unsigned)dk[thr - 1] >> IDX_BITS) == ((unsigned)dk[thr] >> IDX_BITS)) atomic_or_int(&ctl[1], 1);
+                    if (b.tid == 0 && D > thr && ((unsigned)dk[thr - 1] >> IDX_BITS) == ((unsigned)dk[thr] >> IDX_BITS)) {
+                        const unsigned g = (unsigned)dk[thr] >> IDX_BITS;
+                        if (rung == 0) { xf[g] = 1; atomic_or_int(&ctl[vslot], 1); }
+                        else if (!xf[g]) atomic_or_int(&ctl[vslot], 1);
+                    }
+#ifdef OCTA_SIM_KD_PARTIAL_REFUSE
+                    if (b.tid == 0 && rung == 1) atomic_or_int(&ctl[vslot], 1);
+#endif
                     b.sync();
-                    if (ctl[1]) break;
+                    if (rung == 1 && OCTA_UNLIKELY(ctl[vslot])) break;
                 }
                 if (D < thr) break;
                 const int minused = upto > 50000 ? upto * 2 : upto * 4;
@@ -3345,7 +3436,7 @@
             t_key = own;
             set_in_lds = true;
         }
-        if (set_in_lds && (ranked || !ctl[1])) {
+        if (set_in_lds && (rung == 2 || !ctl[vslot])) {
             const int n_co2_0 = sc->n_co2;
             int base = 0;
             {
@@ -3391,15 +3482,18 @@
             int D = 0;
             for (int i = 0; i < n_pairs; i++) {
                 const unsigned pr = A.pairs[i];
-                const int o = ranked ? (int)A.kd_idx[pr & IDX_MASK] : (int)(pr & IDX_MASK);
+                const int o = sink_of(pr);
                 if (!A.ven_near[o]) {
                     const int used = S.used;
                     pyset_add(S, o, A.hashes[o]);
-                    if (!ranked && S.used != used) { cw[D] = o; cw[OCAP + D] = (int)(pr >> IDX_BITS); D++; }
-                }
-            }
-            if (!ranked && !pyset_order_free(cw, cw + OCAP, A.hashes, D, cw + 4 * OCAP, cw + 2 * OCAP, cw + 3 * OCAP, SETCAP / 2)) ctl[1] = 1;
-            if (ranked || !ctl[1]) {
+                    if (rung < 2 && S.used != used) { cw[D] = o; cw[OCAP + D] = (int)(pr >> IDX_BITS); D++; }
+                }
+            }
+            if (rung < 2 && pyset_order_check(cw, cw + OCAP, A.hashes, D, cw + 4 * OCAP, cw + 2 * OCAP, cw + 3 * OCAP, SETCAP / 2, xf, rung == 1)) ctl[vslot] = 1;
+#ifdef OCTA_SIM_KD_PARTIAL_REFUSE
+            if (rung == 1) ctl[vslot] = 1;
+#endif
+            if (rung == 2 || !ctl[vslot]) {
                 int n_co2 = sc->n_co2;
                 for (int e = 0; e <= S.mask; e++)
                     if (S.key[e] >= 0) {
@@ -3413,8 +3507,16 @@
         }
         b.sync();
         OCTA_SUBPROF(sc, 14, t0);
-        if (!ranked && ctl[1]) continue;
-        if (b.tid == 0) sc->kd_path[ranked ? 1 : 0]++;
+        if (rung < 2 && ctl[vslot]) {
+#ifdef OCTA_SIM_KD_NOPARTIAL
+            rung = 2;
+#else
+            from_partial = rung == 1;
+            rung++;
+#endif
+            continue;
+        }
+        if (b.tid == 0) sc->kd_path[rung]++;
         break;
     }
 #if defined(OCTA_SIM_DEBUG_SAT) && !defined(OCTA_SIM_ITER_PROF)
@@ -3428,7 +3530,7 @@
         for (int o = b.tid; o < 2 * n_oxy; o += b.nth) mark[o] = 0;
         b.sync();
         for (int i = b.tid; i < n_pairs; i += b.nth) {
-            const int o = ranked ? (int)A.kd_idx[A.pairs[i] & IDX_MASK] : (int)(A.pairs[i] & IDX_MASK);
+            const int o = sink_of(A.pairs[i]);
             mark[o] = 1;
             if (!A.ven_near[o]) mark[n_oxy + o] = 1;
         }
```

Result: faster. 1544 (median of 6 runs) (+6.6%).
